# LeCAR-Lab/dial-mpc

Hardware: NVIDIA H100
Metric: sample-steps/s (Nsample*Hsample/wall-s) per MPC reverse_once, Go2 (higher is better)
Workload: dtype f32

## Files before the change

### __graft_entry__.py

```python
from __future__ import annotations

import os
import subprocess
import sys

ROOT = os.path.dirname(os.path.abspath(__file__))
CSRC = os.path.join(ROOT, "dial_mpc_b200", "csrc")
LIB = os.path.join(CSRC, "libdial_b200.so")
NVCC_FLAGS = ["-gencode", "arch=compute_90a,code=sm_90a", "-lineinfo", "-O3", "-std=c++17",
              "-use_fast_math", "-Xcompiler", "-fPIC"]
LINK_FLAGS = ["-gencode", "arch=compute_90a,code=sm_90a", "-shared", "-Xcompiler", "-fPIC", "-cudart", "static"]
VARIANTS = (1, 2, 3, 4, 0)
OBJDIR = os.path.join(CSRC, "build")


def _digest(srcs, extra=""):
    import hashlib
    h = hashlib.sha256()
    for s in srcs:
        h.update(open(s, "rb").read())
    h.update((" ".join(NVCC_FLAGS + LINK_FLAGS) + extra).encode())
    return h.hexdigest()


def _stale(target, digest):
    side = target + ".sha256"
    if not (os.path.exists(target) and os.path.exists(side)):
        return True
    return open(side).read().strip() != digest


def _stamp(target, digest):
    with open(target + ".sha256", "w") as f:
        f.write(digest)


def _shape_defines():
    if ROOT not in sys.path:
        sys.path.insert(0, ROOT)
    from dial_mpc_b200.modelc.shape import SHAPES, env_structure_defines
    return [(name, env_structure_defines(env)) for name, env in SHAPES]


def build_library(force: bool = False, extra=(), lib: str = LIB, objdir: str = OBJDIR) -> None:
    extra = list(extra)
    tag = " " + " ".join(extra)
    hdrs = [os.path.join(CSRC, f) for f in ("dial_device.cuh", "dial_host.h")] + [os.path.join(ROOT, "include", "dial_b200.h")]
    var_src = os.path.join(CSRC, "dial_rollout_variant.cu")
    abi_src = os.path.join(CSRC, "dial_kernels.cu")
    shapes = _shape_defines()
    shape_tag = "".join(f" {name}:" + ",".join(d) for name, d in shapes)
    lib_digest = _digest(hdrs + [var_src, abi_src], tag + shape_tag)
    if not (force or _stale(lib, lib_digest)):
        return
    nvcc = os.environ.get("NVCC", "/usr/local/cuda/bin/nvcc")
    os.makedirs(objdir, exist_ok=True)
    jobs = []
    for v in VARIANTS:
        obj = os.path.join(objdir, f"rollout_v{v}.o")
        jobs.append((obj, _digest(hdrs + [var_src], f" variant={v}" + tag),
                     [nvcc] + NVCC_FLAGS + extra + [f"-DDIAL_VARIANT={v}", "-c", "-o", obj, var_src]))
    for name, defs in shapes:
        obj = os.path.join(objdir, f"rollout_{name}.o")
        flags = ["-DDIAL_VARIANT=1", f"-DDIAL_SHAPE_NAME={name}"] + [f"-D{d}" for d in defs]
        jobs.append((obj, _digest(hdrs + [var_src], " " + " ".join(flags) + tag),
                     [nvcc] + NVCC_FLAGS + extra + flags + ["-c", "-o", obj, var_src]))
    obj = os.path.join(objdir, "dial_kernels.o")
    jobs.append((obj, _digest(hdrs + [abi_src], tag), [nvcc] + NVCC_FLAGS + extra + ["-c", "-o", obj, abi_src]))
    running = [(o, d, subprocess.Popen(cmd)) for o, d, cmd in jobs if force or _stale(o, d)]
    for o, d, p in running:
        if p.wait() != 0:
            for _, _, q in running:
                q.wait()
            raise RuntimeError(f"nvcc failed for {o}")
        _stamp(o, d)
    subprocess.check_call([nvcc] + LINK_FLAGS + ["-o", lib] + [o for o, _, _ in jobs])
    _stamp(lib, lib_digest)


def build(force: bool = False) -> None:
    build_library(force)
    if ROOT not in sys.path:
        sys.path.insert(0, ROOT)
    import dial_mpc_b200
    from dial_mpc_b200 import _capi
    _capi.lib()
    ex = os.path.join(ROOT, "dial_mpc_b200", "examples", "custom_env")
    if ex not in sys.path:
        sys.path.insert(0, ex)
    import quadpod_env
    _ = quadpod_env.QuadpodEnv(quadpod_env.QuadpodEnvConfig()).library_path
    from dial_mpc_b200 import custom
    custom.build_library(quadpod_env.QuadpodEnv.reward_source, variant=0)
    import pincher_env
    _ = pincher_env.PincherEnv(pincher_env.PincherEnvConfig()).library_path
    for mod in ("tests.emul.emul", "oracle.build_oracle"):
        path = os.path.join(ROOT, *mod.split(".")) + ".py"
        if os.path.exists(path):
            subprocess.check_call([sys.executable, "-c", f"import {mod} as m; m.build()"], cwd=ROOT)


def smoke() -> None:
    if ROOT not in sys.path:
        sys.path.insert(0, ROOT)
    import numpy as np
    import torch
    build()
    import dial_mpc_b200.envs as E
    from dial_mpc_b200 import random as drandom
    from dial_mpc_b200.core.dial_config import DialConfig
    from dial_mpc_b200.core.dial_core import MBDPI
    from oracle.envs_oracle import make_env
    from oracle.planner_oracle import PlannerOracle
    torch.cuda.set_device(0)
    cfg = DialConfig(env_name="unitree_go2_walk", Nsample=64, Hsample=8, Hnode=4, temp_sample=0.05)
    env = E.get_environment(cfg.env_name, config=E.UnitreeGo2EnvConfig(default_vx=0.8, ramp_up_time=1.0))
    mb = MBDPI(cfg, env)
    state = env.reset(drandom.PRNGKey(0))
    rng = np.random.default_rng(0)
    eps = rng.standard_normal((cfg.Nsample, cfg.Hnode + 1, mb.nu)).astype(np.float32)
    Y0 = torch.zeros(cfg.Hnode + 1, mb.nu, device=mb.device)
    _, Ybar, info = mb.reverse_once(state, drandom.PRNGKey(1), Y0, mb.sigma_control, eps=eps)
    torch.cuda.synchronize()
    o = make_env(cfg.env_name, dict(default_vx=0.8, ramp_up_time=1.0))
    po = PlannerOracle(o, cfg.Nsample, cfg.Hsample, cfg.Hnode, cfg.temp_sample, cfg.horizon_diffuse_factor,
                       cfg.traj_diffuse_factor)
    Yo, io = po.reverse_once(o.reset(), eps.astype(np.float64), np.zeros((cfg.Hnode + 1, mb.nu)), po.sigma_control)
    rews = info["rews"].cpu().numpy()
    err_r = np.abs(rews - io["rews"]).max()
    err_y = np.abs(Ybar.cpu().numpy() - Yo).max()
    print(f"smoke: max|rews - oracle| = {err_r:.3e}, max|Ybar - oracle| = {err_y:.3e}, launches = {mb.plan.launches}")
    assert np.isfinite(rews).all()
    assert err_r < 2e-3 and err_y < 5e-3, "CUDA reverse_once disagrees with the oracle"


if __name__ == "__main__":
    build()
    if len(sys.argv) > 1 and sys.argv[1] == "smoke":
        smoke()
```

### dial_mpc_b200/csrc/dial_kernels.cu

```cuda
#include <cuda_runtime.h>
#include <stdio.h>
#include <stdlib.h>
#include <float.h>
#include <cmath>
#include <memory>
#include <string>
#include <vector>
#include <new>
#include "dial_host.h"
#define DIAL_STR2(x) #x
#define DIAL_STR(x) DIAL_STR2(x)

static thread_local std::string g_err;
static int fail(const std::string& s) { g_err = s; return -1; }
#define CUDA_OK(x) do { cudaError_t e_ = (x); if (e_ != cudaSuccess) return fail(std::string(#x) + ": " + cudaGetErrorString(e_)); } while (0)

#ifdef DIAL_ONLY_VARIANT
#define DIAL_HAS_VARIANT(v) ((v) == DIAL_ONLY_VARIANT)
#define DIAL_VARIANT DIAL_ONLY_VARIANT
#include "dial_rollout_variant.cu"
#else
#define DIAL_HAS_VARIANT(v) 1
#endif
#define DIAL_DECL_LAUNCH(v) cudaError_t dial_launch_rollout_v##v(const DevModel*, const DevPlan*, const RolloutArgs&, int, int, size_t, cudaStream_t);
#if DIAL_HAS_VARIANT(0)
DIAL_DECL_LAUNCH(0)
#endif
#if DIAL_HAS_VARIANT(1)
DIAL_DECL_LAUNCH(1)
#endif
#if DIAL_HAS_VARIANT(2)
DIAL_DECL_LAUNCH(2)
#endif
#if DIAL_HAS_VARIANT(3)
DIAL_DECL_LAUNCH(3)
#endif
#if DIAL_HAS_VARIANT(4)
DIAL_DECL_LAUNCH(4)
#endif
#ifndef DIAL_ONLY_VARIANT
typedef cudaError_t (*dial_launch_fn)(const DevModel*, const DevPlan*, const RolloutArgs&, int, int, size_t, cudaStream_t);
#define DIAL_DECL_SHAPE(s) \
  cudaError_t dial_launch_rollout_##s(const DevModel*, const DevPlan*, const RolloutArgs&, int, int, size_t, cudaStream_t); \
  bool dial_shape_matches_##s(const DevModel&, const dial_plan_desc&);
DIAL_DECL_SHAPE(go2)
static const struct {
  const char* name;
  dial_launch_fn launch;
  bool (*matches)(const DevModel&, const dial_plan_desc&);
} kShapes[] = {{"go2", dial_launch_rollout_go2, dial_shape_matches_go2}};
#endif

template <typename T, int K>
__device__ __forceinline__ void block_reduce(T (&v)[K], T* mx, T* red) {
  const int lane = threadIdx.x & 31, wid = threadIdx.x >> 5, nw = blockDim.x >> 5;
#pragma unroll
  for (int o = 16; o > 0; o >>= 1) {
#pragma unroll
    for (int k = 0; k < K; ++k) v[k] += __shfl_xor_sync(0xffffffffu, v[k], o);
    if (mx) *mx = fmax(*mx, __shfl_xor_sync(0xffffffffu, *mx, o));
  }
  __syncthreads();
  if (lane == 0) {
#pragma unroll
    for (int k = 0; k < K; ++k) red[k * 32 + wid] = v[k];
    if (mx) red[K * 32 + wid] = *mx;
  }
  __syncthreads();
#pragma unroll
  for (int k = 0; k < K; ++k) v[k] = lane < nw ? red[k * 32 + lane] : T(0);
  if (mx) *mx = lane < nw ? red[K * 32 + lane] : T(-INFINITY);
#pragma unroll
  for (int o = 16; o > 0; o >>= 1) {
#pragma unroll
    for (int k = 0; k < K; ++k) v[k] += __shfl_xor_sync(0xffffffffu, v[k], o);
    if (mx) *mx = fmax(*mx, __shfl_xor_sync(0xffffffffu, *mx, o));
  }
}

struct SoftmaxParams {
  float shift, inv, mx;
  bool none;
};
__device__ __noinline__ SoftmaxParams reward_softmax_params_fp64(const float* __restrict__ rews, int n, float temp,
                                                                 float rbar, float mean, float cnt, float* red_f) {
  double* red = reinterpret_cast<double*>(red_f);
  SoftmaxParams s;
  s.none = false;
  const double c = isfinite(mean) ? (double)rbar + (double)mean : 0.0;
  double s1[1] = {0.0}, s2[1] = {0.0}, rmax = -INFINITY;
  for (int i = threadIdx.x; i < n; i += blockDim.x) {
    const float r = __ldcg(rews + i);
    if (isfinite(r)) { const double d = (double)r - c; s1[0] += d; s2[0] += d * d; rmax = fmax(rmax, (double)r); }
  }
  block_reduce<double, 1>(s1, &rmax, red);
  block_reduce<double, 1>(s2, nullptr, red);
  const double m = s1[0] / (double)cnt, var64 = s2[0] / (double)cnt - m * m;
  s.shift = (float)rmax;
  s.mx = 0.f;
  s.inv = var64 > 0.0 ? (float)fmin(1.0 / (sqrt(var64) * (double)temp), 3.4028234663852886e38) : 0.f;
  return s;
}
__device__ __forceinline__ SoftmaxParams reward_softmax_params(const float* __restrict__ rews, int n, float temp,
                                                               float* red) {
  float rbar = __ldcg(rews + n - 1);
  const bool rbar_finite = isfinite(rbar);
  if (!rbar_finite) rbar = 0.f;
  float st[3] = {0.f, 0.f, 0.f}, dmax = -INFINITY;
  for (int i = threadIdx.x; i < n; i += blockDim.x) {
    const float r = __ldcg(rews + i);
    if (isfinite(r)) { const float d = r - rbar; st[0] += 1.f; st[1] += d; st[2] += d * d; dmax = fmaxf(dmax, d); }
  }
  block_reduce<float, 3>(st, &dmax, red);
  SoftmaxParams s;
  const float cnt = st[0];
  s.none = cnt == 0.f;
  const float mean = st[1] / fmaxf(cnt, 1.f);
  const float var = st[2] / fmaxf(cnt, 1.f) - mean * mean;
  const float sd = sqrtf(fmaxf(var, 0.f));
  if (s.none || (rbar_finite && isfinite(st[2]) && fabsf(mean) <= 8.f * sd)) {
    s.shift = rbar;
    s.inv = (sd > 0.f) ? 1.f / sd / temp : 0.f;
    s.mx = dmax * s.inv;
    return s;
  }
  return reward_softmax_params_fp64(rews, n, temp, rbar, mean, cnt, red);
}

struct XchWait {
  const float* mbox;
  const uint32_t* flags;
  uint32_t* seq;
  uint32_t* err;
  float* rews_copy;
  int world;
};
__device__ __forceinline__ unsigned long long globaltimer_ns() {
  unsigned long long t;
  asm volatile("mov.u64 %0, %%globaltimer;" : "=l"(t));
  return t;
}
__device__ __forceinline__ void xch_wait_flags(const uint32_t* flags, uint32_t want, int world, uint32_t* err,
                                               uint32_t* acc = nullptr) {
  if ((int)threadIdx.x < world) {
    const volatile uint32_t* f = flags + threadIdx.x;
    const unsigned long long t0 = globaltimer_ns();
    while (*f < want) {
      if (globaltimer_ns() - t0 > 4000000000ull) { *err = 1u; break; }
      __nanosleep(100);
    }
    if (acc) {
      const unsigned long long dt = globaltimer_ns() - t0;
      const unsigned m = __reduce_max_sync(__activemask(), (unsigned)(dt > 0xffffffffull ? 0xffffffffull : dt));
      if (threadIdx.x == 0) *acc += m;
    }
    __threadfence_system();
  }
  __syncthreads();
}

__global__ void __launch_bounds__(1024) weights_kernel(const float* __restrict__ rews, int n, float temp,
                                                        float* __restrict__ weights, const XchWait X) {
  __shared__ __align__(8) float red[4 * 32];
  const int tid = threadIdx.x;
  if (X.mbox) {
    const uint32_t seq = *X.seq, buf = seq & 1u;
    xch_wait_flags(X.flags + buf * DIAL_MAXRANK, seq + 1u, X.world, X.err, X.err + 2);
    rews = X.mbox + (size_t)buf * n;
    if (X.rews_copy)
      for (int i = tid; i < n; i += blockDim.x) X.rews_copy[i] = __ldcg(rews + i);
  }
  const SoftmaxParams s = reward_softmax_params(rews, n, temp, red);
  if (s.none) {
    for (int i = tid; i < n; i += blockDim.x) weights[i] = (i == n - 1) ? 1.f : 0.f;
    if (X.mbox && tid == 0) *X.seq = *X.seq + 1u;
    return;
  }
  float z[1] = {0.f};
  for (int i = tid; i < n; i += blockDim.x) {
    const float r = __ldcg(rews + i);
    const float e = isfinite(r) ? expf((r - s.shift) * s.inv - s.mx) : 0.f;
    weights[i] = e;
    z[0] += e;
  }
  block_reduce<float, 1>(z, nullptr, red);
  const float iz = 1.f / z[0];
  for (int i = tid; i < n; i += blockDim.x) weights[i] *= iz;
  if (X.mbox && tid == 0) *X.seq = *X.seq + 1u;
}

struct BarsXch {
  float* mbox[DIAL_MAXRANK];
  uint32_t* flags[DIAL_MAXRANK];
  uint32_t* seq;
  uint32_t* err;
  int world, rank, nbar;
  const float* partial;
  float* out[3];
  int n0, n1;
};
__global__ void __launch_bounds__(1024) bars_allreduce_kernel(const BarsXch B) {
  const uint32_t seq = *B.seq, buf = seq & 1u;
  const size_t half = (size_t)buf * DIAL_MAXRANK * B.nbar;
  for (int p = 0; p < B.world; ++p) {
    float* dst = B.mbox[p] + half + (size_t)B.rank * B.nbar;
    for (int i = threadIdx.x; i < B.nbar; i += blockDim.x) dst[i] = B.partial[i];
  }
  __threadfence_system();
  __syncthreads();
  if (threadIdx.x == 0) {
    __threadfence_system();
    for (int p = 0; p < B.world; ++p)
      *reinterpret_cast<volatile uint32_t*>(B.flags[p] + buf * DIAL_MAXRANK + B.rank) = seq + 1u;
  }
  __syncthreads();
  xch_wait_flags(B.flags[B.rank] + buf * DIAL_MAXRANK, seq + 1u, B.world, B.err, B.err + 3);
  const float* mine = B.mbox[B.rank] + half;
  for (int i = threadIdx.x; i < B.nbar; i += blockDim.x) {
    float s_ = 0.f;
    for (int p = 0; p < B.world; ++p) s_ += __ldcg(mine + (size_t)p * B.nbar + i);
    float* o = i < B.n0 ? B.out[0] + i : (i < B.n0 + B.n1 ? B.out[1] + (i - B.n0) : B.out[2] + (i - B.n0 - B.n1));
    *o = s_;
  }
  __syncthreads();
  if (threadIdx.x == 0) *B.seq = seq + 1u;
}

__device__ __forceinline__ float ordered_column_sum(const float* __restrict__ col, int stride, unsigned count, bool on) {
  float tot = 0.f;
  if (!on) return tot;
  unsigned b = 0;
  for (; b + 16 <= count; b += 16) {
    float v[16];
#pragma unroll
    for (int k = 0; k < 16; ++k) v[k] = __ldcg(col + (size_t)(b + k) * stride);
#pragma unroll
    for (int k = 0; k < 16; ++k) tot += v[k];
  }
  for (; b < count; ++b) tot += __ldcg(col + (size_t)b * stride);
  return tot;
}

#define YBAR_THREADS 256
__global__ void __launch_bounds__(YBAR_THREADS) ybar_kernel(const float* __restrict__ weights, const float* __restrict__ eps,
                                                             uint32_t key0, uint32_t key1, const float* __restrict__ Ybar,
                                                             const float* __restrict__ noise, int Ntotal, int Hn1, int nu,
                                                             float* __restrict__ partial, unsigned int* __restrict__ counter,
                                                             float* __restrict__ Ybar_out,
                                                             const uint32_t* __restrict__ key_dev) {
  if (key_dev) { key0 = key_dev[0]; key1 = key_dev[1]; }
  const int ne = Hn1 * nu;
  __shared__ float acc[YBAR_THREADS];
  __shared__ bool is_last;
  const int slots = YBAR_THREADS / ne;
  const int slot = threadIdx.x / ne, el = threadIdx.x - slot * ne;
  float a = 0.f;
  if (slot < slots) {
    const int k = el / nu;
    const float yb = Ybar[el], ns = noise[k];
    const uint32_t ntot = (uint32_t)Ntotal * (uint32_t)ne;
    for (int n = blockIdx.x * slots + slot; n <= Ntotal; n += gridDim.x * slots) {
      float y = yb;
      if (n < Ntotal && k > 0) {
        uint32_t idx = (uint32_t)n * (uint32_t)ne + (uint32_t)el;
        float e = eps ? eps[idx] : jax_normal_legacy(key0, key1, idx, ntot);
        y = e * ns + yb;
      }
      y = fminf(fmaxf(y, -1.f), 1.f);
      a += weights[n] * y;
    }
  }
  acc[threadIdx.x] = a;
  __syncthreads();
  if (threadIdx.x < ne) {
    float s = 0.f;
    for (int sl = 0; sl < slots; ++sl) s += acc[sl * ne + threadIdx.x];
    partial[blockIdx.x * ne + threadIdx.x] = s;
  }
  __threadfence();
  __syncthreads();
  if (threadIdx.x == 0) is_last = (atomicAdd(counter, 1u) == gridDim.x - 1);
  __syncthreads();
  if (is_last) {
    if (threadIdx.x < ne) Ybar_out[threadIdx.x] = ordered_column_sum(partial + threadIdx.x, ne, gridDim.x, true);
    if (threadIdx.x == 0) *counter = 0u;
  }
}

__global__ void __launch_bounds__(YBAR_THREADS) update_kernel(const float* __restrict__ rews, int n, float temp,
                                                               float* __restrict__ weights, const XchWait X,
                                                               uint32_t* __restrict__ rng, const float* __restrict__ Ybar,
                                                               const float* __restrict__ noise, int Ntotal, int Hn1, int nu,
                                                               float* __restrict__ partial, unsigned int* __restrict__ counter,
                                                               float* __restrict__ Ybar_out, const InstSchedule* __restrict__ sched,
                                                               const int32_t* __restrict__ iter_lim, int iter,
                                                               const float* weights_prev) {
  __shared__ __align__(8) float red[4 * 32];
  __shared__ float acc[YBAR_THREADS];
  __shared__ bool is_last;
  const int tid = threadIdx.x;
  {
    const size_t b = blockIdx.y, ne1 = (size_t)Hn1 * nu;
    rews += b * n; weights += b * n; rng += 2 * b; Ybar += b * ne1; Ybar_out += b * ne1;
    partial += b * gridDim.x * (ne1 + 1); counter += b;
    if (!schedule_runs(iter_lim, b, iter)) {
      if (blockIdx.x == 0)
        for (int i = tid; i < (int)ne1; i += blockDim.x) Ybar_out[i] = Ybar[i];
      if (weights_prev != weights - b * n)
        for (int i = blockIdx.x * blockDim.x + tid; i < n; i += gridDim.x * blockDim.x) weights[i] = weights_prev[b * n + i];
      return;
    }
    if (sched && sched[b].on) { temp = sched[b].temp; noise = sched[b].noise[iter]; }
  }
  if (X.mbox) {
    const uint32_t seq = *X.seq, buf = seq & 1u;
    xch_wait_flags(X.flags + buf * DIAL_MAXRANK, seq + 1u, X.world, X.err, blockIdx.x == 0 ? X.err + 2 : nullptr);
    rews = X.mbox + (size_t)buf * n;
  }
  uint32_t key0, key1;
  const uint32_t r0 = rng[0], r1 = rng[1];
  split_key(r0, r1, key0, key1);
  const SoftmaxParams sp = reward_softmax_params(rews, n, temp, red);
  const int ne = Hn1 * nu;
  const int slots = YBAR_THREADS / ne;
  const int slot = tid / ne, el = tid - slot * ne;
  float a = 0.f, z = 0.f;
  if (slot < slots) {
    const int k = el / nu;
    const float yb = Ybar[el], ns = noise[k];
    const uint32_t ntot = (uint32_t)Ntotal * (uint32_t)ne;
    for (int s_ = blockIdx.x * slots + slot; s_ <= Ntotal; s_ += gridDim.x * slots) {
      const float r = __ldcg(rews + s_);
      float e = isfinite(r) ? expf((r - sp.shift) * sp.inv - sp.mx) : 0.f;
      if (sp.none) e = (s_ == Ntotal) ? 1.f : 0.f;
      float y = yb;
      if (s_ < Ntotal && k > 0) {
        const uint32_t idx = (uint32_t)s_ * (uint32_t)ne + (uint32_t)el;
        y = jax_normal_legacy(key0, key1, idx, ntot) * ns + yb;
      }
      y = fminf(fmaxf(y, -1.f), 1.f);
      a += e * y;
      if (el == 0) { z += e; weights[s_] = e; }
    }
  }
  acc[tid] = a;
  float zz[1] = {z};
  block_reduce<float, 1>(zz, nullptr, red);
  __syncthreads();
  if (tid < ne) {
    float s_ = 0.f;
    for (int sl = 0; sl < slots; ++sl) s_ += acc[sl * ne + tid];
    partial[blockIdx.x * (ne + 1) + tid] = s_;
  }
  if (tid == 0) partial[blockIdx.x * (ne + 1) + ne] = zz[0];
  __threadfence();
  __syncthreads();
  if (tid == 0) is_last = (atomicAdd(counter, 1u) == gridDim.x - 1);
  __syncthreads();
  if (!is_last) return;
  __threadfence();
  __shared__ float zsh;
  float tot = ordered_column_sum(partial + tid, ne + 1, gridDim.x, tid <= ne);
  if (tid == ne) zsh = tot;
  if (ne == (int)blockDim.x && tid == 0) zsh = ordered_column_sum(partial + ne, ne + 1, gridDim.x, true);
  __syncthreads();
  const float iz = 1.f / zsh;
  if (tid < ne) Ybar_out[tid] = tot * iz;
  for (int i = tid; i < n; i += blockDim.x) {
    weights[i] = __ldcg(weights + i) * iz;
    if (X.mbox && X.rews_copy) X.rews_copy[i] = __ldcg(rews + i);
  }
  if (tid == 0) {
    *counter = 0u;
    uint32_t n0, n1;
    split_rng(r0, r1, n0, n1);
    rng[0] = n0; rng[1] = n1;
    if (X.mbox) *X.seq = *X.seq + 1u;
  }
}

__global__ void mpc_split_kernel(uint32_t* __restrict__ rng, uint32_t* __restrict__ key) {
  if (threadIdx.x == 0) {
    const uint32_t k0 = rng[0], k1 = rng[1];
    uint32_t a0 = 0, b0 = 2, a1 = 1, b1 = 3;
    threefry2x32(k0, k1, a0, b0);
    threefry2x32(k0, k1, a1, b1);
    rng[0] = a0; rng[1] = a1; key[0] = b0; key[1] = b1;
  }
}

__global__ void mpc_shift_kernel(const float* __restrict__ Msh, const float* __restrict__ Yin,
                                 float* __restrict__ Yout, int n1, int nu) {
  const int i = threadIdx.x;
  Yin += (size_t)blockIdx.x * n1 * nu; Yout += (size_t)blockIdx.x * n1 * nu;
  if (i < n1 * nu) {
    const int k = i / nu, a = i - k * nu;
    float s = 0.f;
    for (int j = 0; j < n1; ++j) s += Msh[k * n1 + j] * Yin[j * nu + a];
    Yout[i] = s;
  }
}

#define TB_CHUNKS 32
struct TrajArgs {
  const float* traj[3];
  float* out[3];
  int ncol[3], coloff[3];
  int coltot, nrows, H;
  int inst_rows;
  const float* weights;
  int w_offset, mean_row, mean_weight_index, include_mean;
  float* partial;
};

template <bool BATCH>
__global__ void __launch_bounds__(256, 8) trajbar_partial_kernel(const TrajArgs T, const int32_t* __restrict__ iter_lim, int iter) {
  const int chunk = blockIdx.y, arr = BATCH ? blockIdx.z % 3 : blockIdx.z, inst = BATCH ? blockIdx.z / 3 : 0;
  const int ncol = arr == 0 ? T.ncol[0] : (arr == 1 ? T.ncol[1] : T.ncol[2]), len = T.H * ncol;
  const int coloff = arr == 0 ? T.coloff[0] : (arr == 1 ? T.coloff[1] : T.coloff[2]);
  const int j = blockIdx.x * 256 + threadIdx.x;
  if (blockIdx.x * 256 >= len || (BATCH && !schedule_runs(iter_lim, inst, iter))) return;
  const float* __restrict__ traj = (arr == 0 ? T.traj[0] : (arr == 1 ? T.traj[1] : T.traj[2])) + (size_t)inst * T.inst_rows * len;
  const float* wts = BATCH ? T.weights + (size_t)inst * (T.mean_weight_index + 1) : T.weights;
  const int per = (T.nrows + TB_CHUNKS - 1) / TB_CHUNKS;
  const int r0 = chunk * per, r1 = min(T.nrows, r0 + per);
  const int jj = j < len ? j : len - 1;
  float a = 0.f;
  for (int r = r0; r < r1; r += 8) {
    float wv[8], xv[8];
#pragma unroll
    for (int k = 0; k < 8; ++k) {
      const int rr = r + k;
      float wgt = 0.f;
      if (rr < r1) {
        if (rr == T.mean_row) wgt = T.include_mean ? wts[T.mean_weight_index] : 0.f;
        else wgt = wts[T.w_offset + rr];
      }
      wv[k] = wgt;
    }
#pragma unroll
    for (int k = 0; k < 8; ++k)
      xv[k] = (wv[k] != 0.f) ? traj[(size_t)(r + k) * len + jj] : 0.f;
#pragma unroll
    for (int k = 0; k < 8; ++k) a += wv[k] * xv[k];
  }
  if (j < len) {
    const int t = j / ncol, c = j - t * ncol;
    T.partial[(((size_t)inst * TB_CHUNKS + chunk) * T.H + t) * T.coltot + coloff + c] = a;
  }
}

template <bool BATCH>
__global__ void __launch_bounds__(128, 8) trajbar_final_kernel(const TrajArgs T, const int32_t* __restrict__ iter_lim, int iter) {
  const int t = blockIdx.x, inst = BATCH ? blockIdx.y : 0;
  if (BATCH && !schedule_runs(iter_lim, inst, iter)) return;
  const float* partial = T.partial + (size_t)inst * TB_CHUNKS * T.H * T.coltot;
  for (int col = threadIdx.x; col < T.coltot; col += blockDim.x) {
    float s = 0.f;
#pragma unroll 8
    for (int ch = 0; ch < TB_CHUNKS; ++ch) s += partial[((size_t)ch * T.H + t) * T.coltot + col];
    float* out; int ncol, off;
    if (col >= T.coloff[2]) { out = T.out[2]; ncol = T.ncol[2]; off = T.coloff[2]; }
    else if (col >= T.coloff[1]) { out = T.out[1]; ncol = T.ncol[1]; off = T.coloff[1]; }
    else { out = T.out[0]; ncol = T.ncol[0]; off = T.coloff[0]; }
    if (out) out[((size_t)inst * T.H + t) * ncol + (col - off)] = s;
  }
}

__global__ void __launch_bounds__(256) ensemble_reduce_kernel(const float* __restrict__ r, const EnsRisk* __restrict__ risk,
                                                              const EnsAdapt* __restrict__ adapt, const float* __restrict__ belief,
                                                              int K, int n1, float* __restrict__ rews,
                                                              const int32_t* __restrict__ iter_lim, int iter) {
  const int i = blockIdx.x * blockDim.x + threadIdx.x, b = blockIdx.y;
  if (i >= n1 || !schedule_runs(iter_lim, b, iter)) return;
  const EnsRisk R = risk[b];
  const float* rb = r + (size_t)b * K * n1 + i;
  rews[(size_t)b * n1 + i] = adapt[b].on ? ens_risk_reduce_weighted(rb, (size_t)n1, K, R, belief + (size_t)b * K, adapt[b].prune)
                                         : ens_risk_reduce(rb, (size_t)n1, K, R);
}

__global__ void __launch_bounds__(128) ens_gather_kernel(const float* __restrict__ Y, int K, int n1, int nu,
                                                         float* __restrict__ us) {
  const int b = blockIdx.x;
  for (int i = threadIdx.x; i < K * nu; i += blockDim.x) us[(size_t)b * K * nu + i] = Y[(size_t)b * n1 * nu + i % nu];
}

__global__ void __launch_bounds__(32) ens_belief_kernel(const float* __restrict__ vhat, const float* __restrict__ qvel,
                                                        const EnsAdapt* __restrict__ adapt, int K, int nv,
                                                        double* __restrict__ L, float* __restrict__ w, float* __restrict__ ell) {
  const int b = blockIdx.x, lane = threadIdx.x;
  if (!adapt[b].on) return;
  __shared__ double l[DIAL_MAXENS];
  if (lane < K) {
    l[lane] = ens_member_loglik(vhat + ((size_t)b * K + lane) * nv, qvel + (size_t)b * nv, adapt[b].sigma, nv);
    ell[(size_t)b * K + lane] = (float)l[lane];
  }
  __syncwarp();
  if (lane == 0) ens_belief_update(L + (size_t)b * K, w + (size_t)b * K, l, K, (double)adapt[b].forget);
}

__global__ void __launch_bounds__(128) delay_queue_kernel(const DelaySetting* __restrict__ set, int32_t* __restrict__ head,
                                                          float* __restrict__ ring, const float* __restrict__ Y, int n1,
                                                          int nu, int pop, float* __restrict__ applied,
                                                          float* __restrict__ pending, int32_t* __restrict__ pred_len) {
  const int b = blockIdx.x;
  const DelaySetting s = set[b];
  const int h = head[b];
  const size_t q = (size_t)b * DIAL_MAXDELAY * nu;
  const int h1 = delay_queue_step(ring + q, h, s.d, nu, Y + (size_t)b * n1 * nu, applied + (size_t)b * nu, pending + q,
                                  pop != 0, threadIdx.x, blockDim.x);
  __syncthreads();
  if (threadIdx.x == 0) { head[b] = h1; pred_len[b] = s.predict && s.d > 0 ? s.d : 0; }
}

__global__ void __launch_bounds__(128) delay_refill_kernel(int b, int d, int32_t* __restrict__ head, float* __restrict__ ring,
                                                           const float* __restrict__ Y, int n1, int nu,
                                                           float* __restrict__ pending) {
  const size_t q = (size_t)b * DIAL_MAXDELAY * nu;
  const float* y0 = Y + (size_t)b * n1 * nu;
  for (int a = threadIdx.x; a < nu; a += blockDim.x)
    for (int j = 0; j < d; ++j) ring[q + (size_t)j * nu + a] = y0[a];
  delay_queue_step(ring + q, 0, d, nu, y0, nullptr, pending + q, false, threadIdx.x, blockDim.x);
  if (threadIdx.x == 0) head[b] = 0;
}

struct ObsBuffers {
  ObsRing* ring;
  float *rq, *rv, *rw, *ra;
  int32_t* rc;
  float *oq, *ov, *ow;
  int32_t *oc, *age;
  float* seq;
  int32_t* len;
};

__global__ void __launch_bounds__(128) observe_kernel(const DevModel* __restrict__ M, const ObsSetting* __restrict__ set,
                                                      ObsBuffers O, const DelaySetting* __restrict__ dset,
                                                      const float* __restrict__ pending, int env_step,
                                                      const float* __restrict__ qpos, const float* __restrict__ qvel,
                                                      const float* __restrict__ warm, const int32_t* __restrict__ cnt,
                                                      const float* __restrict__ act, int act_row, float* __restrict__ pq,
                                                      float* __restrict__ pv, float* __restrict__ pw, int32_t* __restrict__ pc) {
  const int b = blockIdx.x;
  const dial_model_desc& m = M->m;
  const size_t nq = m.nq, nv = m.nv, nu = m.nu, R = DIAL_OBSRING;
  const ObsSetting& s = set[b];
  const ObsRing r = O.ring[b];
  const DelaySetting ds = dset ? dset[b] : DelaySetting{0, 0};
  const ObsRing r1 = observe_advance(s, r, env_step != 0);
  ObsView V;
  V.qpos = qpos + b * nq; V.qvel = qvel + b * nv; V.warm = warm + b * nv; V.cnt = cnt + 2 * b;
  V.act = env_step ? act + b * act_row : nullptr;
  V.rq = O.rq + b * R * nq; V.rv = O.rv + b * R * nv; V.rw = O.rw + b * R * nv; V.ra = O.ra + b * R * nu;
  V.rc = O.rc + b * R * 2;
  V.oq = O.oq + b * nq; V.ov = O.ov + b * nv; V.ow = O.ow + b * nv; V.oc = O.oc + 2 * b;
  V.pq = pq + b * nq; V.pv = pv + b * nv; V.pw = pw + b * nv; V.pc = pc + 2 * b;
  V.seq = O.seq + b * DIAL_MAXDELAY * nu;
  V.pending = pending ? pending + b * DIAL_MAXDELAY * nu : nullptr;
  observe_record(observe_pushes(s, r, env_step != 0), r1, V, (int)nq, (int)nv, (int)nu, threadIdx.x, blockDim.x);
  __syncthreads();
  observe_emit(s, r1, m, ds.d, V, threadIdx.x, blockDim.x);
  if (threadIdx.x == 0) {
    const int age = observe_age(s, r1);
    O.ring[b] = r1; O.age[b] = age; O.len[b] = ds.predict ? age + ds.d : 0;
  }
}

__global__ void observe_reset_kernel(int b, const ObsSetting* __restrict__ set, ObsRing* __restrict__ ring) {
  ObsRing r;
  r.head = 0; r.count = 0;
  r.key[0] = set[b].key[0]; r.key[1] = set[b].key[1]; r.sub[0] = 0u; r.sub[1] = 0u;
  ring[b] = r;
}

template <class T> struct Staged {
  T* d = nullptr;
  T* h = nullptr;
  size_t width = 1;
  std::vector<cudaEvent_t> ev;
  cudaError_t allocate(size_t n, size_t w, const T& init) {
    width = w;
    cudaError_t e = cudaMallocHost(&h, n * w * sizeof(T));
    if (e == cudaSuccess) e = cudaMalloc(&d, n * w * sizeof(T));
    if (e == cudaSuccess) {
      for (size_t i = 0; i < n * w; ++i) h[i] = init;
      e = cudaMemcpy(d, h, n * w * sizeof(T), cudaMemcpyHostToDevice);
    }
    if (e != cudaSuccess) { release(); return e; }
    ev.assign(n, nullptr);
    return cudaSuccess;
  }
  template <class F> cudaError_t put(size_t s, F fill, cudaStream_t st) {
    cudaEvent_t& e_s = ev[s];
    cudaError_t e = e_s ? cudaEventSynchronize(e_s) : cudaEventCreateWithFlags(&e_s, cudaEventDisableTiming);
    if (e == cudaSuccess) {
      fill(h + s * width);
      e = cudaMemcpyAsync(d + s * width, h + s * width, width * sizeof(T), cudaMemcpyHostToDevice, st);
    }
    if (e == cudaSuccess) e = cudaEventRecord(e_s, st);
    return e;
  }
  void release() {
    for (cudaEvent_t e : ev) if (e) cudaEventDestroy(e);
    ev.clear();
    cudaFree(d); cudaFreeHost(h);
    d = nullptr; h = nullptr;
  }
};

struct LaunchKey {
  bool models = false, members = false, sched = false, lims = false, adapt = false, delay = false, obs = false;
  bool predicts = false;
  int npred = 0;
  bool planning() const { return obs || npred > 0; }
  bool operator!=(const LaunchKey& o) const {
    return models != o.models || members != o.members || sched != o.sched || lims != o.lims || adapt != o.adapt ||
           delay != o.delay || obs != o.obs || predicts != o.predicts || npred != o.npred;
  }
};

struct dial_plan {
  DevModel hM;
  DevPlan hP;
  DevModel* dM = nullptr;
  DevPlan* dP = nullptr;
  int variant = 0;
  int shape = 0;
  int n_inst = 1;
  int n_ens = 0;
  int num_sms = 132;
  size_t smem_bytes = 0;
  float *traj_q[2] = {nullptr, nullptr}, *traj_qd[2] = {nullptr, nullptr}, *traj_x[2] = {nullptr, nullptr};
  int cur = 0;
  float* weights = nullptr;
  float* weights2 = nullptr;
  cudaStream_t side = nullptr;
  cudaEvent_t ev_main[2] = {nullptr, nullptr}, ev_side[2] = {nullptr, nullptr};
  float* partial = nullptr;
  float* tb_partial = nullptr;
  unsigned int* counter = nullptr;
  unsigned int* row_counter = nullptr;
  float* zeros = nullptr;
  int ybar_grid = 0;
  int upd_grid = 0;
  int64_t launches = 0;
  float* dbg = nullptr;
  dial_mpc_buffers mpc{};
  bool mpc_bound = false;
  float* mpc_Msh = nullptr;
  float* mpc_Y1 = nullptr;
  uint32_t* mpc_key = nullptr;
  struct MpcGraph { int n_diffuse, env_step, seen; cudaGraphExec_t exec; int64_t launches; };
  std::vector<MpcGraph> mpc_graphs;
  LaunchKey key, ran;
  Staged<DevModel> models;
  Staged<DevModel> members;
  float* ens_rews = nullptr;
  Staged<EnsRisk> risk;
  Staged<EnsAdapt> adapt;
  Staged<double> belief_L;
  Staged<float> belief_w;
  float* dEll = nullptr;
  float* pred_us = nullptr;
  float* pred_qd = nullptr;
  Staged<InstSchedule> sched;
  Staged<int32_t> lims;
  struct PlanningState {
    float *qpos = nullptr, *qvel = nullptr, *warm = nullptr;
    int32_t* cnt = nullptr;
    DevModel* models = nullptr;
  } planning;
  Staged<DelaySetting> delay;
  struct DelayQueue {
    int32_t* head = nullptr;
    float *ring = nullptr, *applied = nullptr, *pending = nullptr;
    int32_t* len = nullptr;
  } queue;
  Staged<ObsSetting> obs;
  ObsBuffers ob{};
  std::vector<void**> owned;
  template <class T> cudaError_t own(cudaError_t& e, T*& ptr, size_t bytes, bool zero = false, cudaStream_t st = nullptr) {
    void** slot = reinterpret_cast<void**>(&ptr);
    if (e == cudaSuccess && (e = cudaMalloc(slot, bytes)) == cudaSuccess) owned.push_back(slot);
    if (e == cudaSuccess && zero) e = cudaMemsetAsync(ptr, 0, bytes, st);
    return e;
  }
  void free_since(size_t mark) {
    for (; owned.size() > mark; owned.pop_back()) { cudaFree(*owned.back()); *owned.back() = nullptr; }
  }
  struct Exchange {
    bool on = false;
    int rank = 0, world = 1, nbar = 0;
    uint32_t* base[DIAL_MAXRANK] = {nullptr};
    size_t words = 0, o_mbox = 0, o_bars = 0, o_flags = 0, o_bflags = 0, o_local = 0;
    float* bars_partial = nullptr;
    float* mbox(int p) const { return reinterpret_cast<float*>(base[p] + o_mbox); }
    float* bars(int p) const { return reinterpret_cast<float*>(base[p] + o_bars); }
    uint32_t* flags(int p) const { return base[p] + o_flags; }
    uint32_t* bflags(int p) const { return base[p] + o_bflags; }
    uint32_t* seq() const { return base[rank] + o_local; }
    unsigned int* done() const { return base[rank] + o_local + 1; }
    uint32_t* err() const { return base[rank] + o_local + 2; }
    uint32_t* bseq() const { return base[rank] + o_local + 3; }
  } xch;
};

static void drop_graphs(dial_plan* p) {
  for (auto& g : p->mpc_graphs) if (g.exec) cudaGraphExecDestroy(g.exec);
  p->mpc_graphs.clear();
}

static LaunchKey launch_key(const dial_plan* p) {
  LaunchKey k;
  k.models = p->models.d != nullptr; k.members = p->members.d != nullptr;
  k.sched = p->sched.d != nullptr; k.lims = p->lims.d != nullptr; k.adapt = p->pred_qd != nullptr;
  k.delay = p->delay.d != nullptr; k.obs = p->obs.d != nullptr;
  for (int b = 0; k.delay && b < p->n_inst; ++b) {
    const DelaySetting& s = p->delay.h[b];
    const int n = s.d + (k.obs && p->obs.h[b].on ? p->obs.h[b].k : 0);
    if (!s.predict) continue;
    k.predicts |= s.d > 0;
    k.npred = n > k.npred ? n : k.npred;
  }
  return k;
}

static void fill_xch(const dial_plan* p, RolloutArgs& A) {
  if (!p->xch.on) return;
  A.xch_world = p->xch.world; A.xch_rank = p->xch.rank;
  for (int r = 0; r < p->xch.world; ++r) { A.xch_mbox[r] = p->xch.mbox(r); A.xch_flags[r] = p->xch.flags(r); }
  A.xch_seq = p->xch.seq(); A.xch_done = p->xch.done();
}
static XchWait xch_wait_args(const dial_plan* p, float* rews_copy) {
  XchWait X; memset(&X, 0, sizeof(X));
  if (p->xch.on) {
    X.mbox = p->xch.mbox(p->xch.rank); X.flags = p->xch.flags(p->xch.rank); X.seq = p->xch.seq(); X.err = p->xch.err();
    X.rews_copy = rews_copy; X.world = p->xch.world;
  }
  return X;
}

extern "C" int dial_abi_version(void) { return DIAL_ABI_VERSION; }
extern "C" const char* dial_last_error(void) { return g_err.c_str(); }
extern "C" size_t dial_sizeof(int which) {
  return which == 0 ? sizeof(dial_model_desc) : which == 1 ? sizeof(dial_plan_desc) : which == 2 ? sizeof(dial_state)
       : which == 3 ? sizeof(dial_mpc_buffers) : which == 4 ? sizeof(dial_task) : 0;
}

static cudaError_t launch_rollout(dial_plan* p, const RolloutArgs& A, int wpc, cudaStream_t st) {
  const size_t smem = sizeof(DevModel) + sizeof(DevPlan) + (size_t)wpc * p->hM.warp_floats * sizeof(float);
  int grid = (A.nrows + wpc - 1) / wpc;
  if (A.models && model_rows(A) > 0) grid = (A.nrows / model_rows(A)) * ((model_rows(A) + wpc - 1) / wpc);
  if (A.row_counter) {
    const int resident = p->num_sms * (wpc > 8 ? 1 : 16 / wpc);
    grid = grid < resident ? grid : resident;
    cudaError_t e = cudaMemsetAsync(A.row_counter, 0, sizeof(unsigned int), st);
    if (e != cudaSuccess) return e;
  }
  p->launches++;
#ifndef DIAL_ONLY_VARIANT
  if (p->shape > 0) return kShapes[p->shape - 1].launch(p->dM, p->dP, A, grid, wpc, smem, st);
#endif
  switch (p->variant) {
#if DIAL_HAS_VARIANT(1)
    case 1: return dial_launch_rollout_v1(p->dM, p->dP, A, grid, wpc, smem, st);
#endif
#if DIAL_HAS_VARIANT(2)
    case 2: return dial_launch_rollout_v2(p->dM, p->dP, A, grid, wpc, smem, st);
#endif
#if DIAL_HAS_VARIANT(3)
    case 3: return dial_launch_rollout_v3(p->dM, p->dP, A, grid, wpc, smem, st);
#endif
#if DIAL_HAS_VARIANT(4)
    case 4: return dial_launch_rollout_v4(p->dM, p->dP, A, grid, wpc, smem, st);
#endif
#if DIAL_HAS_VARIANT(0)
    case 0: return dial_launch_rollout_v0(p->dM, p->dP, A, grid, wpc, smem, st);
#endif
    default: return cudaErrorInvalidDeviceFunction;
  }
}

static int default_wpc(const dial_plan* p, int nrows) {
  const int per_sm = (nrows + p->num_sms - 1) / p->num_sms;
  const size_t fixed = sizeof(DevModel) + sizeof(DevPlan), slab = (size_t)p->hM.warp_floats * sizeof(float);
  int maxw = DIAL_MAXTHREADS / 32;
  while (maxw > 1 && fixed + maxw * slab > 227 * 1024) --maxw;
  if (per_sm <= maxw) return per_sm;
  const int waves = (per_sm + maxw - 1) / maxw;
  return (per_sm + waves - 1) / waves;
}

static cudaError_t launch_rollout_any(dial_plan* p, const RolloutArgs& A0, cudaStream_t st) {
  RolloutArgs A = A0;
  const char* f = getenv("DIAL_WPC");
  int wpc = f ? atoi(f) : 0;
  if (wpc == 0) {
    wpc = default_wpc(p, A.nrows);
    if (A.models && model_rows(A) > 0) {
      const int cpi = (model_rows(A) + wpc - 1) / wpc;
      wpc = (model_rows(A) + cpi - 1) / cpi;
    }
  }
  if (wpc < 1 || wpc > DIAL_MAXTHREADS / 32) return cudaErrorInvalidValue;
  A.lockstep = (wpc >= 2 && !getenv("DIAL_NO_LOCKSTEP")) ? 1 : 0;
  if (p->hM.dense && !A.lockstep && !A.models && A.nrows > wpc * p->num_sms && !getenv("DIAL_NO_DYNAMIC_ROWS")) A.row_counter = p->row_counter;
  const bool mid = getenv("DIAL_MIDSYNC") ? true : (getenv("DIAL_NO_MIDSYNC") ? false : (p->hM.dense || !p->hM.s_on));
  if (A.lockstep && mid) A.lockstep = 2;
  { const char* se = getenv("DIAL_SYNC_EVERY"); A.sync_every = se ? atoi(se) : 1; if (A.sync_every < 1) A.sync_every = 1; }
  const char* dl = getenv("DIAL_DENSE_LOCKSTEP");
  if (A.lockstep == 2 && p->hM.dense && !(dl && atoi(dl) == 2)) A.lockstep = 3;
  return launch_rollout(p, A, wpc, st);
}

extern "C" dial_plan* dial_plan_create(const dial_model_desc* model, const dial_plan_desc* cfg) {
  if (!model || !cfg) { g_err = "null descriptor"; return nullptr; }
  dial_plan* p = new (std::nothrow) dial_plan();
  if (!p) { g_err = "out of memory"; return nullptr; }
  std::string err;
  if (!derive_model(*model, p->hM, err)) { g_err = err; delete p; return nullptr; }
  {
    int dev = 0, sms = 0;
    if (cudaGetDevice(&dev) == cudaSuccess && cudaDeviceGetAttribute(&sms, cudaDevAttrMultiProcessorCount, dev) == cudaSuccess && sms > 0)
      p->num_sms = sms;
  }
  p->variant = (getenv("DIAL_FORCE_GENERIC_TREE") && !p->hM.dense) ? 0 : star_variant(p->hM);
  if (p->variant < 0) { g_err = "this build instantiates the dense (elliptic) solver path for nv = " DIAL_STR(DIAL_DENSE_NV) " only (custom builds: dial_mpc_b200.custom compiles it for the model's nv)"; delete p; return nullptr; }
  memset(&p->hP, 0, sizeof(DevPlan));
  p->hP.c = *cfg;
  p->hP.c.cmd_step = -1;
  const dial_plan_desc& c = *cfg;
  if (c.Hsample + 1 > DIAL_MAXH || c.Hnode + 1 > DIAL_MAXNODE || c.Hnode < 1 || c.Nsample < 1 || c.Ntotal < c.Nsample ||
      c.n_frames < 1 || (c.Hnode + 1) * model->nu > YBAR_THREADS || c.n_stage > DIAL_MAXSTAGE) {
    g_err = "invalid plan configuration (Hsample/Hnode/Nsample/n_frames out of range)";
    delete p;
    return nullptr;
  }
  if (c.env_id < DIAL_ENV_GO2_WALK || c.env_id > DIAL_ENV_CUSTOM) { g_err = "unknown env_id"; delete p; return nullptr; }
#ifndef DIAL_CUSTOM_REWARD_FILE
  if (c.env_id == DIAL_ENV_CUSTOM) {
    g_err = "env_id DIAL_ENV_CUSTOM needs a library built with a reward source (dial_mpc_b200.custom.build_library); this is the stock build";
    delete p; return nullptr;
  }
#endif
#ifdef DIAL_ONLY_VARIANT
  if (p->variant != DIAL_ONLY_VARIANT) {
    g_err = "this custom build holds solver variant " + std::to_string(DIAL_ONLY_VARIANT) + " only, the model needs " + std::to_string(p->variant);
    delete p; return nullptr;
  }
#endif
  if (c.n_user < 0 || c.n_user > DIAL_MAXUSER) { g_err = "n_user out of range"; delete p; return nullptr; }
  if (c.n_inst < 0) { g_err = "n_inst must be >= 0 (0 or 1: a single instance)"; delete p; return nullptr; }
  if (c.n_inst > 1) {
    if (c.Ntotal != c.Nsample) { g_err = "a batched plan (n_inst > 1) cannot be sharded (Ntotal must equal Nsample)"; delete p; return nullptr; }
    if (c.Nsample + 1 > (1 << 17)) { g_err = "a batched plan (n_inst > 1) needs Nsample + 1 <= 131072 (the fused update)"; delete p; return nullptr; }
    if (c.n_inst > 65535 / 3 || (int64_t)c.n_inst * (c.Nsample + 1) > 0x7fffffff) {
      g_err = "n_inst too large: at most 21845 instances and 2^31 - 1 rows per rollout launch"; delete p; return nullptr;
    }
  }
  p->n_inst = c.n_inst > 1 ? c.n_inst : 1;
  if (c.n_ens < 0 || c.n_ens > DIAL_MAXENS) { g_err = "n_ens out of range (0..DIAL_MAXENS = " DIAL_STR(DIAL_MAXENS) ")"; delete p; return nullptr; }
  if (c.n_ens >= 1) {
    if (c.Ntotal != c.Nsample) { g_err = "an ensemble plan (n_ens >= 1) cannot be sharded (Ntotal must equal Nsample)"; delete p; return nullptr; }
    if ((int64_t)p->n_inst * c.n_ens * (c.Nsample + 1) > 0x7fffffff) { g_err = "n_inst * n_ens * (Nsample + 1) exceeds 2^31 - 1 rows per rollout launch"; delete p; return nullptr; }
  }
  p->n_ens = c.n_ens;
#ifndef DIAL_ONLY_VARIANT
  if (p->variant == 1 && !getenv("DIAL_FORCE_GENERIC_SHAPE"))
    for (int s = 0; s < (int)(sizeof(kShapes) / sizeof(kShapes[0])); ++s)
      if (kShapes[s].matches(p->hM, p->hP.c)) { p->shape = s + 1; break; }
#endif
  auto bad = [&](cudaError_t e, const char* what) {
    g_err = std::string(what) + ": " + cudaGetErrorString(e);
    dial_plan_destroy(p);
    return (dial_plan*)nullptr;
  };
  cudaError_t e = cudaSuccess;
  if (p->own(e, p->dM, sizeof(DevModel)) != cudaSuccess) return bad(e, "cudaMalloc(model)");
  if (p->own(e, p->dP, sizeof(DevPlan)) != cudaSuccess) return bad(e, "cudaMalloc(plan)");
  if ((e = cudaMemcpy(p->dM, &p->hM, sizeof(DevModel), cudaMemcpyHostToDevice)) != cudaSuccess) return bad(e, "cudaMemcpy(model)");
  if ((e = cudaMemcpy(p->dP, &p->hP, sizeof(DevPlan), cudaMemcpyHostToDevice)) != cudaSuccess) return bad(e, "cudaMemcpy(plan)");
  const size_t B = (size_t)p->n_inst, H = (size_t)c.Hsample + 1;
  const size_t rows = B * (p->n_ens > 1 ? (size_t)p->n_ens : 1) * ((size_t)c.Nsample + 1);
  const dial_model_desc& m = *model;
  for (int b = 0; b < 2; ++b) {
    if (p->own(e, p->traj_q[b], rows * H * m.nq * sizeof(float)) != cudaSuccess) return bad(e, "cudaMalloc(traj_q)");
    if (p->own(e, p->traj_qd[b], rows * H * m.nv * sizeof(float)) != cudaSuccess) return bad(e, "cudaMalloc(traj_qd)");
    if (p->own(e, p->traj_x[b], rows * H * 3 * (m.nbody - 1) * sizeof(float)) != cudaSuccess) return bad(e, "cudaMalloc(traj_x)");
  }
  if (p->n_ens > 1) {
    if (p->own(e, p->ens_rews, rows * sizeof(float)) != cudaSuccess) return bad(e, "cudaMalloc(ens_rews)");
    const size_t K = p->n_ens;
    const double L0 = log(1.0 / p->n_ens);
    if ((e = p->risk.allocate(B, 1, ens_risk_derive(p->n_ens, DIAL_ENS_MEAN, 1.f))) != cudaSuccess) return bad(e, "allocate(risk)");
    if ((e = p->adapt.allocate(B, 1, EnsAdapt{})) != cudaSuccess) return bad(e, "allocate(adapt)");
    if ((e = p->belief_L.allocate(B, K, L0)) != cudaSuccess) return bad(e, "allocate(belief)");
    if ((e = p->belief_w.allocate(B, K, (float)exp(L0))) != cudaSuccess) return bad(e, "allocate(belief)");
    if (p->own(e, p->dEll, B * K * sizeof(float)) != cudaSuccess) return bad(e, "cudaMalloc(belief)");
    if ((e = cudaMemset(p->dEll, 0, B * K * sizeof(float))) != cudaSuccess) return bad(e, "cudaMemset(belief)");
  }
  if (p->own(e, p->weights, B * ((size_t)c.Ntotal + 1) * sizeof(float)) != cudaSuccess) return bad(e, "cudaMalloc(weights)");
  if (p->own(e, p->weights2, B * ((size_t)c.Ntotal + 1) * sizeof(float)) != cudaSuccess) return bad(e, "cudaMalloc(weights2)");
  if ((e = cudaStreamCreateWithFlags(&p->side, cudaStreamNonBlocking)) != cudaSuccess) return bad(e, "cudaStreamCreate(side)");
  for (int i = 0; i < 2; ++i) {
    if ((e = cudaEventCreateWithFlags(&p->ev_main[i], cudaEventDisableTiming)) != cudaSuccess) return bad(e, "cudaEventCreate");
    if ((e = cudaEventCreateWithFlags(&p->ev_side[i], cudaEventDisableTiming)) != cudaSuccess) return bad(e, "cudaEventCreate");
  }
  const int ne = (c.Hnode + 1) * m.nu, slots = YBAR_THREADS / ne;
  int g = (c.Ntotal + 1 + slots - 1) / slots;
  p->ybar_grid = g < 1 ? 1 : (g > 2 * p->num_sms ? 2 * p->num_sms : g);
  {
    int gu = (c.Ntotal + 1 + slots * 8 - 1) / (slots * 8);
    p->upd_grid = gu < 1 ? 1 : (gu > p->ybar_grid ? p->ybar_grid : gu);
  }
  if (p->own(e, p->partial, B * p->ybar_grid * (ne + 1) * sizeof(float)) != cudaSuccess) return bad(e, "cudaMalloc(partial)");
  if (p->own(e, p->tb_partial, B * TB_CHUNKS * H * (m.nq + m.nv + 3 * (m.nbody - 1)) * sizeof(float)) != cudaSuccess) return bad(e, "cudaMalloc(tb_partial)");
  if (p->own(e, p->counter, B * sizeof(unsigned int)) != cudaSuccess) return bad(e, "cudaMalloc(counter)");
  if ((e = cudaMemset(p->counter, 0, B * sizeof(unsigned int))) != cudaSuccess) return bad(e, "cudaMemset(counter)");
  if (p->own(e, p->row_counter, sizeof(unsigned int)) != cudaSuccess) return bad(e, "cudaMalloc(row_counter)");
  if (getenv("DIAL_DEBUG_COUNTERS")) {
    if (p->own(e, p->dbg, 8 * sizeof(float)) != cudaSuccess) return bad(e, "cudaMalloc(dbg)");
    cudaMemset(p->dbg, 0, 8 * sizeof(float));
  }
  if (p->own(e, p->zeros, DIAL_MAXV * sizeof(float)) != cudaSuccess) return bad(e, "cudaMalloc(zeros)");
  if ((e = cudaMemset(p->zeros, 0, DIAL_MAXV * sizeof(float))) != cudaSuccess) return bad(e, "cudaMemset(zeros)");
  return p;
}

extern "C" void dial_plan_destroy(dial_plan* p) {
  if (!p) return;
  drop_graphs(p);
  for (int r = 0; r < DIAL_MAXRANK; ++r) {
    if (!p->xch.base[r]) continue;
    if (r == p->xch.rank) cudaFree(p->xch.base[r]); else cudaIpcCloseMemHandle(p->xch.base[r]);
  }
  cudaFree(p->xch.bars_partial);
  p->models.release(); p->members.release(); p->risk.release();
  p->adapt.release(); p->belief_L.release(); p->belief_w.release(); p->sched.release(); p->lims.release();
  p->delay.release(); p->obs.release();
  for (int i = 0; i < 2; ++i) { if (p->ev_main[i]) cudaEventDestroy(p->ev_main[i]); if (p->ev_side[i]) cudaEventDestroy(p->ev_side[i]); }
  if (p->side) cudaStreamDestroy(p->side);
  p->free_since(0);
  delete p;
}

static void fill_state(RolloutArgs& A, const dial_state* s) {
  A.qpos0 = s->qpos; A.qvel0 = s->qvel; A.warm0 = s->qacc_warmstart; A.step0 = s->step; A.stage0 = s->stage;
}

extern "C" int dial_rollout(dial_plan* p, const dial_state* s, const float* us, int B, int H, float* rewss,
                            float* q, float* qd, float* xpos, void* stream) {
  if (!p || !s || !us || !rewss) return fail("dial_rollout: null argument");
  if (B < 1 || H < 1) return fail("dial_rollout: B and H must be positive");
  RolloutArgs A; memset(&A, 0, sizeof(A));
  fill_state(A, s);
  A.nrows = B; A.H = H; A.mode = 0; A.us = us; A.rewss = rewss; A.q = q; A.qd = qd; A.xpos = xpos;
  CUDA_OK(launch_rollout_any(p, A, (cudaStream_t)stream));
  return 0;
}

extern "C" int dial_plan_set_command(dial_plan* p, int cmd_step, const float* vel, const float* ang, void* stream) {
  if (!p) return fail("dial_plan_set_command: null plan");
  if (cmd_step >= 0 && (!vel || !ang)) return fail("dial_plan_set_command: null command");
  dial_plan_desc& c = p->hP.c;
  c.cmd_step = cmd_step;
  for (int i = 0; i < 3; ++i) { c.cmd_vel[i] = cmd_step >= 0 ? vel[i] : 0.f; c.cmd_ang[i] = cmd_step >= 0 ? ang[i] : 0.f; }
  const size_t off = offsetof(dial_plan_desc, cmd_step);
  CUDA_OK(cudaMemcpyAsync((char*)p->dP + off, (const char*)&p->hP.c + off, sizeof(int32_t) + 6 * sizeof(float),
                          cudaMemcpyHostToDevice, (cudaStream_t)stream));
  return 0;
}

extern "C" int dial_plan_set_stages(dial_plan* p, int n_stage, const float* pose_seq, const float* yaw_seq,
                                    const float* contact_targets, const float* contact_radius, void* stream) {
  if (!p) return fail("dial_plan_set_stages: null plan");
  if (n_stage < 1 || n_stage > DIAL_MAXSTAGE) return fail("dial_plan_set_stages: n_stage out of range (1..DIAL_MAXSTAGE)");
  if (!pose_seq || !yaw_seq || !contact_targets || !contact_radius) return fail("dial_plan_set_stages: null table");
  dial_plan_desc& c = p->hP.c;
  c.n_stage = n_stage;
  memset(c.pose_seq, 0, sizeof(c.pose_seq)); memset(c.yaw_seq, 0, sizeof(c.yaw_seq));
  memset(c.contact_targets, 0, sizeof(c.contact_targets)); memset(c.contact_radius, 0, sizeof(c.contact_radius));
  memcpy(c.pose_seq, pose_seq, sizeof(float) * 3 * n_stage);
  memcpy(c.yaw_seq, yaw_seq, sizeof(float) * n_stage);
  memcpy(c.contact_targets, contact_targets, sizeof(float) * 12 * n_stage);
  memcpy(c.contact_radius, contact_radius, sizeof(float) * 4 * n_stage);
  const size_t off = offsetof(dial_plan_desc, n_stage), end = offsetof(dial_plan_desc, n_user);
  CUDA_OK(cudaMemcpyAsync((char*)p->dP + off, (const char*)&p->hP.c + off, end - off, cudaMemcpyHostToDevice,
                          (cudaStream_t)stream));
  return 0;
}

static std::string fmt_g(double x) {
  char buf[64];
  snprintf(buf, sizeof(buf), "%g", x);
  return buf;
}

static int need_ensemble(const dial_plan* p, const char* fn, int k) {
  if (!p) return fail(std::string(fn) + ": null plan");
  if (p->n_ens >= k) return 0;
  if (k == 1) return fail(std::string(fn) + ": the plan has no ensemble (dial_plan_desc.n_ens = 0)");
  return fail(std::string(fn) + ": the plan needs an ensemble of n_ens >= " + std::to_string(k) + " members, it has " + std::to_string(p->n_ens));
}
static int need_instance(const dial_plan* p, const char* fn, int b) {
  if (b >= 0 && b < p->n_inst) return 0;
  return fail(std::string(fn) + ": instance " + std::to_string(b) + " out of range (0.." + std::to_string(p->n_inst - 1) + ")");
}

static int set_model_slot(dial_plan* p, const char* fn, Staged<DevModel>& a, size_t n, size_t slot,
                          const dial_model_desc* m, cudaStream_t st) {
  std::unique_ptr<DevModel> D(new (std::nothrow) DevModel());
  if (!D) return fail("out of memory");
  std::string err;
  if (!derive_model(*m, *D, err)) return fail(std::string(fn) + ": " + err);
  if (const char* diff = instance_model_difference(p->hM, *D))
    return fail(std::string(fn) + ": field '" + diff + "' differs from the plan's model "
                "(an instance's model may differ in floats other than timestep, jnt_range and actuator_ctrlrange only)");
  cudaError_t e = cudaSuccess;
  if (!a.d && (e = a.allocate(n, 1, p->hM)) != cudaSuccess) return fail(std::string(fn) + ": " + cudaGetErrorString(e));
  e = a.put(slot, [&](DevModel* h) { *h = *D; }, st);
  p->key = launch_key(p);
  CUDA_OK(e);
  return 0;
}

extern "C" int dial_plan_set_instance_model(dial_plan* p, int b, const dial_model_desc* m, void* stream) {
  static const char* fn = "dial_plan_set_instance_model";
  if (!p || !m) return fail(std::string(fn) + ": null argument");
  if (int rc = need_instance(p, fn, b)) return rc;
  if (p->hP.c.Ntotal != p->hP.c.Nsample) return fail(std::string(fn) + ": sharded plans (Ntotal != Nsample) share one model");
  return set_model_slot(p, fn, p->models, (size_t)p->n_inst, (size_t)b, m, (cudaStream_t)stream);
}

extern "C" int dial_plan_set_ensemble_model(dial_plan* p, int b, int k, const dial_model_desc* m, void* stream) {
  static const char* fn = "dial_plan_set_ensemble_model";
  if (!p || !m) return fail(std::string(fn) + ": null argument");
  if (int rc = need_ensemble(p, fn, 1)) return rc;
  if (int rc = need_instance(p, fn, b)) return rc;
  if (k < 0 || k >= p->n_ens) return fail(std::string(fn) + ": member " + std::to_string(k) + " out of range (0.." + std::to_string(p->n_ens - 1) + ")");
  const size_t slot = (size_t)b * p->n_ens + k;
  if (int rc = set_model_slot(p, fn, p->members, (size_t)p->n_inst * p->n_ens, slot, m, (cudaStream_t)stream)) return rc;
  if (k == 0 && p->planning.models)
    CUDA_OK(cudaMemcpyAsync(p->planning.models + b, p->members.d + slot, sizeof(DevModel), cudaMemcpyDeviceToDevice, (cudaStream_t)stream));
  return 0;
}

extern "C" int dial_plan_set_ensemble_risk(dial_plan* p, int b, int mode, float alpha, void* stream) {
  static const char* fn = "dial_plan_set_ensemble_risk";
  if (int rc = need_ensemble(p, fn, 1)) return rc;
  if (int rc = need_instance(p, fn, b)) return rc;
  if (mode != DIAL_ENS_MEAN && mode != DIAL_ENS_CVAR)
    return fail(std::string(fn) + ": mode " + std::to_string(mode) + " is neither DIAL_ENS_MEAN (0) nor DIAL_ENS_CVAR (1)");
  if (mode == DIAL_ENS_CVAR && !(alpha > 0.f && alpha <= 1.f))
    return fail(std::string(fn) + ": alpha must be finite and in (0, 1] for DIAL_ENS_CVAR, got " + fmt_g(alpha));
  if (p->n_ens < 2) return 0;
  cudaError_t e = p->risk.put(b, [&](EnsRisk* r) { *r = ens_risk_derive(p->n_ens, mode, alpha); }, (cudaStream_t)stream);
  if (e != cudaSuccess) return fail(std::string(fn) + ": " + cudaGetErrorString(e));
  return 0;
}

extern "C" int dial_plan_member_rewards(dial_plan* p, float* out, void* stream) {
  static const char* fn = "dial_plan_member_rewards";
  if (!p || !out) return fail(std::string(fn) + ": null argument");
  if (int rc = need_ensemble(p, fn, 1)) return rc;
  if (!p->mpc_bound) return fail(std::string(fn) + ": call dial_mpc_bind first");
  const size_t n = (size_t)p->n_inst * p->n_ens * ((size_t)p->hP.c.Nsample + 1);
  const float* src = p->n_ens > 1 ? p->ens_rews : p->mpc.rews;
  CUDA_OK(cudaMemcpyAsync(out, src, n * sizeof(float), cudaMemcpyDeviceToDevice, (cudaStream_t)stream));
  return 0;
}

extern "C" int dial_plan_set_ensemble_adapt(dial_plan* p, int b, int on, float forget, float prune, const float* sigma, void* stream) {
  static const char* fn = "dial_plan_set_ensemble_adapt";
  if (int rc = need_ensemble(p, fn, 2)) return rc;
  if (int rc = need_instance(p, fn, b)) return rc;
  if (on != 0 && on != 1) return fail(std::string(fn) + ": on must be 0 or 1, got " + std::to_string(on));
  const int K = p->n_ens, nv = p->hM.m.nv;
  if (on) {
    if (!(forget > 0.f && forget <= 1.f)) return fail(std::string(fn) + ": forget must be in (0, 1], got " + fmt_g(forget));
    if (!(prune >= 0.f && (double)prune < 1.0 / K))
      return fail(std::string(fn) + ": prune must be in [0, 1/K) = [0, " + fmt_g(1.0 / K) + "), got " + fmt_g(prune));
    if (!sigma) return fail(std::string(fn) + ": null sigma");
    for (int j = 0; j < nv; ++j)
      if (!(sigma[j] > 0.f && sigma[j] <= FLT_MAX))
        return fail(std::string(fn) + ": sigma[" + std::to_string(j) + "] must be finite and > 0, got " + fmt_g(sigma[j]));
  }
  cudaStream_t st = (cudaStream_t)stream;
  cudaError_t e = cudaSuccess;
  if (on && !p->pred_qd) {
    const size_t rows = (size_t)p->n_inst * K, mark = p->owned.size();
    p->own(e, p->pred_us, rows * p->hM.m.nu * sizeof(float));
    if (p->own(e, p->pred_qd, rows * nv * sizeof(float)) != cudaSuccess) {
      p->free_since(mark);
      return fail(std::string(fn) + ": " + cudaGetErrorString(e));
    }
  }
  e = p->adapt.put(b, [&](EnsAdapt* a) {
    a->on = on;
    if (on) {
      a->forget = forget; a->prune = prune;
      for (int j = 0; j < DIAL_MAXV; ++j) a->sigma[j] = j < nv ? sigma[j] : 1.f;
    }
  }, st);
  p->key = launch_key(p);
  if (e != cudaSuccess) return fail(std::string(fn) + ": " + cudaGetErrorString(e));
  return 0;
}

extern "C" int dial_plan_set_ensemble_belief(dial_plan* p, int b, const float* w, void* stream) {
  static const char* fn = "dial_plan_set_ensemble_belief";
  if (int rc = need_ensemble(p, fn, 2)) return rc;
  if (int rc = need_instance(p, fn, b)) return rc;
  if (!w) return fail(std::string(fn) + ": null w");
  const int K = p->n_ens;
  double sum = 0.0;
  for (int k = 0; k < K; ++k) {
    if (!(w[k] >= 0.f && w[k] <= FLT_MAX)) return fail(std::string(fn) + ": w[" + std::to_string(k) + "] must be finite and >= 0, got " + fmt_g(w[k]));
    sum += (double)w[k];
  }
  if (!(sum > 0.0)) return fail(std::string(fn) + ": the weights must have a positive sum");
  cudaStream_t st = (cudaStream_t)stream;
  cudaError_t e = p->belief_L.put(b, [&](double* L) {
    for (int k = 0; k < K; ++k) L[k] = w[k] > 0.f ? log((double)w[k] / sum) : -INFINITY;
  }, st);
  const double* L = p->belief_L.h + (size_t)b * K;
  if (e == cudaSuccess) e = p->belief_w.put(b, [&](float* W) {
    for (int k = 0; k < K; ++k) W[k] = (float)exp(L[k]);
  }, st);
  if (e != cudaSuccess) return fail(std::string(fn) + ": " + cudaGetErrorString(e));
  return 0;
}

extern "C" int dial_plan_ensemble_belief(dial_plan* p, float* w, float* loglik, void* stream) {
  if (int rc = need_ensemble(p, "dial_plan_ensemble_belief", 2)) return rc;
  const size_t n = (size_t)p->n_inst * p->n_ens * sizeof(float);
  cudaStream_t st = (cudaStream_t)stream;
  if (w) CUDA_OK(cudaMemcpyAsync(w, p->belief_w.d, n, cudaMemcpyDeviceToDevice, st));
  if (loglik) CUDA_OK(cudaMemcpyAsync(loglik, p->dEll, n, cudaMemcpyDeviceToDevice, st));
  return 0;
}

static int need_schedulable(const dial_plan* p, const char* fn) {
  const dial_plan_desc& c = p->hP.c;
  if (c.Ntotal != c.Nsample) return fail(std::string(fn) + ": sharded plans (Ntotal != Nsample) share the plan's schedule");
  if (c.Ntotal + 1 > (1 << 17)) return fail(std::string(fn) + ": needs Ntotal + 1 <= 131072 (the fused update)");
  return 0;
}

extern "C" int dial_plan_set_instance_schedule(dial_plan* p, int b, float temp, int n_rows, const float* noise, void* stream) {
  static const char* fn = "dial_plan_set_instance_schedule";
  if (!p) return fail(std::string(fn) + ": null plan");
  if (int rc = need_instance(p, fn, b)) return rc;
  if (int rc = need_schedulable(p, fn)) return rc;
  const int n1 = p->hP.c.Hnode + 1;
  if (noise) {
    if (!(temp > 0.f && temp <= FLT_MAX)) return fail(std::string(fn) + ": temp must be finite and > 0, got " + fmt_g(temp));
    if (n_rows < 1 || n_rows > DIAL_MAXDIFFUSE)
      return fail(std::string(fn) + ": n_rows " + std::to_string(n_rows) + " out of range (1.." DIAL_STR(DIAL_MAXDIFFUSE) ")");
    for (int i = 0; i < n_rows * n1; ++i)
      if (!(fabsf(noise[i]) <= FLT_MAX))
        return fail(std::string(fn) + ": noise[" + std::to_string(i / n1) + "][" + std::to_string(i % n1) + "] is not finite, got " + fmt_g(noise[i]));
  } else if (!p->sched.d) {
    return 0;
  }
  cudaStream_t st = (cudaStream_t)stream;
  cudaError_t e = cudaSuccess;
  if (!p->sched.d && (e = p->sched.allocate(p->n_inst, 1, InstSchedule{})) != cudaSuccess)
    return fail(std::string(fn) + ": " + cudaGetErrorString(e));
  e = p->sched.put(b, [&](InstSchedule* S) {
    memset(S, 0, sizeof(*S));
    if (!noise) return;
    S->on = 1; S->temp = temp; S->n_rows = n_rows;
    for (int r = 0; r < n_rows; ++r)
      for (int k = 0; k < n1; ++k) S->noise[r][k] = noise[r * n1 + k];
  }, st);
  p->key = launch_key(p);
  if (e != cudaSuccess) return fail(std::string(fn) + ": " + cudaGetErrorString(e));
  return 0;
}

extern "C" int dial_plan_set_instance_iterations(dial_plan* p, const int32_t* n_iter, void* stream) {
  static const char* fn = "dial_plan_set_instance_iterations";
  if (!p || !n_iter) return fail(std::string(fn) + ": null argument");
  if (int rc = need_schedulable(p, fn)) return rc;
  for (int b = 0; b < p->n_inst; ++b)
    if (n_iter[b] < 0 || n_iter[b] > DIAL_MAXDIFFUSE)
      return fail(std::string(fn) + ": n_iter[" + std::to_string(b) + "] = " + std::to_string(n_iter[b]) + " out of range (0.." DIAL_STR(DIAL_MAXDIFFUSE) ")");
  cudaStream_t st = (cudaStream_t)stream;
  cudaError_t e = cudaSuccess;
  if (!p->lims.d) {
    Staged<DevModel>& M = p->n_ens > 0 ? p->members : p->models;
    if (!M.d) e = M.allocate((size_t)p->n_inst * (p->n_ens > 0 ? p->n_ens : 1), 1, p->hM);
    if (e == cudaSuccess) e = p->lims.allocate(1, p->n_inst, DIAL_MAXDIFFUSE);
    if (e != cudaSuccess) return fail(std::string(fn) + ": " + cudaGetErrorString(e));
  }
  e = p->lims.put(0, [&](int32_t* L) { memcpy(L, n_iter, sizeof(int32_t) * p->n_inst); }, st);
  p->key = launch_key(p);
  if (e != cudaSuccess) return fail(std::string(fn) + ": " + cudaGetErrorString(e));
  return 0;
}

static cudaError_t allocate_planning(dial_plan* p, cudaStream_t st) {
  dial_plan::PlanningState& P = p->planning;
  if (P.qpos) return cudaSuccess;
  const size_t B = (size_t)p->n_inst, nq = p->hM.m.nq, nv = p->hM.m.nv;
  cudaError_t e = cudaSuccess;
  p->own(e, P.qpos, B * nq * sizeof(float), true, st);
  p->own(e, P.qvel, B * nv * sizeof(float), true, st);
  p->own(e, P.warm, B * nv * sizeof(float), true, st);
  p->own(e, P.cnt, B * 2 * sizeof(int32_t), true, st);
  if (p->n_ens > 0) p->own(e, P.models, B * sizeof(DevModel));
  for (size_t b = 0; P.models && b < B && e == cudaSuccess; ++b)
    e = p->members.d ? cudaMemcpyAsync(P.models + b, p->members.d + b * p->n_ens, sizeof(DevModel), cudaMemcpyDeviceToDevice, st)
                     : cudaMemcpy(P.models + b, &p->hM, sizeof(DevModel), cudaMemcpyHostToDevice);
  return e;
}

static cudaError_t allocate_delay(dial_plan* p, cudaStream_t st) {
  const size_t B = (size_t)p->n_inst, nu = p->hM.m.nu, mark = p->owned.size();
  dial_plan::DelayQueue& Q = p->queue;
  cudaError_t e = allocate_planning(p, st);
  if (e == cudaSuccess) e = p->delay.allocate(B, 1, DelaySetting{0, 0});
  p->own(e, Q.head, B * sizeof(int32_t), true, st);
  p->own(e, Q.ring, B * DIAL_MAXDELAY * nu * sizeof(float), true, st);
  p->own(e, Q.applied, B * nu * sizeof(float), true, st);
  p->own(e, Q.pending, B * DIAL_MAXDELAY * nu * sizeof(float), true, st);
  p->own(e, Q.len, B * sizeof(int32_t), true, st);
  if (e != cudaSuccess) { p->delay.release(); p->free_since(mark); }
  return e;
}

static cudaError_t allocate_observation(dial_plan* p, cudaStream_t st) {
  const size_t B = (size_t)p->n_inst, nq = p->hM.m.nq, nv = p->hM.m.nv, nu = p->hM.m.nu, R = DIAL_OBSRING;
  const size_t mark = p->owned.size();
  cudaError_t e = allocate_planning(p, st);
  ObsSetting off;
  memset(&off, 0, sizeof(off));
  if (e == cudaSuccess) e = p->obs.allocate(B, 1, off);
  ObsBuffers& O = p->ob;
  p->own(e, O.ring, B * sizeof(ObsRing), true, st);
  p->own(e, O.rq, B * R * nq * sizeof(float), true, st);
  p->own(e, O.rv, B * R * nv * sizeof(float), true, st);
  p->own(e, O.rw, B * R * nv * sizeof(float), true, st);
  p->own(e, O.ra, B * R * nu * sizeof(float), true, st);
  p->own(e, O.rc, B * R * 2 * sizeof(int32_t), true, st);
  p->own(e, O.oq, B * nq * sizeof(float), true, st);
  p->own(e, O.ov, B * nv * sizeof(float), true, st);
  p->own(e, O.ow, B * nv * sizeof(float), true, st);
  p->own(e, O.oc, B * 2 * sizeof(int32_t), true, st);
  p->own(e, O.age, B * sizeof(int32_t), true, st);
  p->own(e, O.seq, B * DIAL_MAXDELAY * nu * sizeof(float), true, st);
  p->own(e, O.len, B * sizeof(int32_t), true, st);
  if (e != cudaSuccess) { p->obs.release(); p->free_since(mark); }
  return e;
}

extern "C" int dial_plan_set_instance_delay(dial_plan* p, int b, int steps, int predict, void* stream) {
  static const char* fn = "dial_plan_set_instance_delay";
  if (!p) return fail(std::string(fn) + ": null plan");
  if (int rc = need_instance(p, fn, b)) return rc;
  const dial_plan_desc& c = p->hP.c;
  if (c.Ntotal != c.Nsample || p->xch.on) return fail(std::string(fn) + ": sharded plans (Ntotal != Nsample) have no per-instance delay");
  if (steps < 0 || steps > DIAL_MAXDELAY)
    return fail(std::string(fn) + ": steps " + std::to_string(steps) + " out of range (0.." DIAL_STR(DIAL_MAXDELAY) ")");
  if (predict != 0 && predict != 1) return fail(std::string(fn) + ": predict must be 0 or 1, got " + std::to_string(predict));
  if (p->obs.d && steps + p->obs.h[b].k > DIAL_MAXDELAY)
    return fail(std::string(fn) + ": steps " + std::to_string(steps) + " plus instance " + std::to_string(b) +
                "'s observation delay " + std::to_string(p->obs.h[b].k) + " exceeds " DIAL_STR(DIAL_MAXDELAY));
  if (!p->mpc_bound) return fail(std::string(fn) + ": call dial_mpc_bind first (the queue is filled from the bound Y)");
  cudaStream_t st = (cudaStream_t)stream;
  cudaError_t e = cudaSuccess;
  if (!p->delay.d && (e = allocate_delay(p, st)) != cudaSuccess) return fail(std::string(fn) + ": " + cudaGetErrorString(e));
  e = p->delay.put(b, [&](DelaySetting* s) { s->d = steps; s->predict = predict; }, st);
  p->key = launch_key(p);
  if (e != cudaSuccess) return fail(std::string(fn) + ": " + cudaGetErrorString(e));
  const int n1 = c.Hnode + 1, nu = p->hM.m.nu;
  delay_refill_kernel<<<1, 128, 0, st>>>(b, steps, p->queue.head, p->queue.ring, p->mpc.Y, n1, nu, p->queue.pending);
  CUDA_OK(cudaGetLastError());
  return 0;
}

extern "C" int dial_plan_set_instance_observation(dial_plan* p, int b, int delay, const float* qpos_std,
                                                  const float* qvel_std, const uint32_t key[2], void* stream) {
  static const char* fn = "dial_plan_set_instance_observation";
  if (!p) return fail(std::string(fn) + ": null plan");
  if (int rc = need_instance(p, fn, b)) return rc;
  if (delay < 0 || delay > DIAL_MAXDELAY)
    return fail(std::string(fn) + ": delay " + std::to_string(delay) + " out of range (0.." DIAL_STR(DIAL_MAXDELAY) ")");
  const int d = p->delay.d ? p->delay.h[b].d : 0;
  if (delay + d > DIAL_MAXDELAY)
    return fail(std::string(fn) + ": delay " + std::to_string(delay) + " plus instance " + std::to_string(b) +
                "'s action delay " + std::to_string(d) + " exceeds " DIAL_STR(DIAL_MAXDELAY));
  const int nv = p->hM.m.nv;
  bool noisy = false;
  for (int w = 0; w < 2; ++w) {
    const float* sd = w == 0 ? qpos_std : qvel_std;
    for (int i = 0; sd && i < nv; ++i) {
      if (!(sd[i] >= 0.f) || !std::isfinite(sd[i]))
        return fail(std::string(fn) + ": " + (w == 0 ? "qpos_std[" : "qvel_std[") + std::to_string(i) + "] = " +
                    std::to_string(sd[i]) + " must be finite and >= 0");
      noisy |= sd[i] != 0.f;
    }
  }
  const dial_plan_desc& c = p->hP.c;
  if (c.Ntotal != c.Nsample || p->xch.on) return fail(std::string(fn) + ": sharded plans (Ntotal != Nsample) have no per-instance observation");
  if (!p->mpc_bound) return fail(std::string(fn) + ": call dial_mpc_bind first");
  cudaStream_t st = (cudaStream_t)stream;
  cudaError_t e = cudaSuccess;
  if (!p->obs.d && (e = allocate_observation(p, st)) != cudaSuccess) return fail(std::string(fn) + ": " + cudaGetErrorString(e));
  e = p->obs.put(b, [&](ObsSetting* s) {
    s->k = delay; s->on = delay > 0 || noisy;
    s->key[0] = key ? key[0] : 0u; s->key[1] = key ? key[1] : 0u;
    for (int i = 0; i < 2 * DIAL_MAXV; ++i) s->sigma[i] = 0.f;
    for (int i = 0; i < nv; ++i) { s->sigma[i] = qpos_std ? qpos_std[i] : 0.f; s->sigma[nv + i] = qvel_std ? qvel_std[i] : 0.f; }
  }, st);
  p->key = launch_key(p);
  if (e != cudaSuccess) return fail(std::string(fn) + ": " + cudaGetErrorString(e));
  observe_reset_kernel<<<1, 1, 0, st>>>(b, p->obs.d, p->ob.ring);
  CUDA_OK(cudaGetLastError());
  return 0;
}

extern "C" int dial_plan_observed_state(dial_plan* p, float* qpos, float* qvel, float* warm, int32_t* counters,
                                        int32_t* age, void* stream) {
  static const char* fn = "dial_plan_observed_state";
  if (!p) return fail(std::string(fn) + ": null plan");
  if (!p->mpc_bound) return fail(std::string(fn) + ": call dial_mpc_bind first");
  const size_t B = (size_t)p->n_inst, nq = p->hM.m.nq, nv = p->hM.m.nv;
  const bool ob = p->ran.obs;
  cudaStream_t st = (cudaStream_t)stream;
  const auto cp = [&](void* dst, const void* src, size_t bytes) {
    return dst ? cudaMemcpyAsync(dst, src, bytes, cudaMemcpyDeviceToDevice, st) : cudaSuccess;
  };
  CUDA_OK(cp(qpos, ob ? p->ob.oq : p->mpc.qpos, B * nq * sizeof(float)));
  CUDA_OK(cp(qvel, ob ? p->ob.ov : p->mpc.qvel, B * nv * sizeof(float)));
  CUDA_OK(cp(warm, ob ? p->ob.ow : p->mpc.qacc_warmstart, B * nv * sizeof(float)));
  CUDA_OK(cp(counters, ob ? p->ob.oc : p->mpc.counters, B * 2 * sizeof(int32_t)));
  if (age) {
    if (ob) CUDA_OK(cp(age, p->ob.age, B * sizeof(int32_t)));
    else CUDA_OK(cudaMemsetAsync(age, 0, B * sizeof(int32_t), st));
  }
  return 0;
}

extern "C" int dial_plan_pending_actions(dial_plan* p, float* out, void* stream) {
  static const char* fn = "dial_plan_pending_actions";
  if (!p || !out) return fail(std::string(fn) + ": null argument");
  const size_t n = (size_t)p->n_inst * DIAL_MAXDELAY * p->hM.m.nu * sizeof(float);
  cudaStream_t st = (cudaStream_t)stream;
  if (p->queue.pending) CUDA_OK(cudaMemcpyAsync(out, p->queue.pending, n, cudaMemcpyDeviceToDevice, st));
  else CUDA_OK(cudaMemsetAsync(out, 0, n, st));
  return 0;
}

extern "C" int dial_plan_planning_state(dial_plan* p, float* qpos, float* qvel, float* warm, int32_t* counters, void* stream) {
  static const char* fn = "dial_plan_planning_state";
  if (!p) return fail(std::string(fn) + ": null plan");
  if (!p->mpc_bound) return fail(std::string(fn) + ": call dial_mpc_bind first");
  const size_t B = (size_t)p->n_inst, nq = p->hM.m.nq, nv = p->hM.m.nv;
  const bool pred = p->ran.planning();
  cudaStream_t st = (cudaStream_t)stream;
  const auto cp = [&](void* dst, const void* src, size_t bytes) {
    return dst ? cudaMemcpyAsync(dst, src, bytes, cudaMemcpyDeviceToDevice, st) : cudaSuccess;
  };
  const dial_plan::PlanningState& P = p->planning;
  CUDA_OK(cp(qpos, pred ? P.qpos : p->mpc.qpos, B * nq * sizeof(float)));
  CUDA_OK(cp(qvel, pred ? P.qvel : p->mpc.qvel, B * nv * sizeof(float)));
  CUDA_OK(cp(warm, pred ? P.warm : p->mpc.qacc_warmstart, B * nv * sizeof(float)));
  CUDA_OK(cp(counters, pred ? P.cnt : p->mpc.counters, B * 2 * sizeof(int32_t)));
  return 0;
}

extern "C" int dial_plan_get_task(const dial_plan* p, dial_task* out) {
  if (!p || !out) return fail("dial_plan_get_task: null argument");
  const dial_task& t = plan_task(p->hP.c);
  if (!task_valid(t)) return fail("dial_plan_get_task: the plan's n_stage / n_user are out of range (1..DIAL_MAXSTAGE / 0..DIAL_MAXUSER)");
  *out = t;
  return 0;
}

extern "C" int dial_env_step(dial_plan* p, const dial_state* s, const float* action, float* qpos_out,
                             float* qvel_out, float* warm_out, float* reward, float* ctrl_out, void* stream) {
  return dial_env_step_kin(p, s, action, qpos_out, qvel_out, warm_out, reward, ctrl_out, nullptr, stream);
}

extern "C" int dial_env_step_kin(dial_plan* p, const dial_state* s, const float* action, float* qpos_out,
                                 float* qvel_out, float* warm_out, float* reward, float* ctrl_out, float* kin_out,
                                 void* stream) {
  if (!p || !s || !action || !qpos_out || !qvel_out || !warm_out || !reward) return fail("dial_env_step: null argument");
  RolloutArgs A; memset(&A, 0, sizeof(A));
  fill_state(A, s);
  A.nrows = 1; A.H = 1; A.mode = 0; A.us = action; A.rewss = reward;
  A.qpos_out = qpos_out; A.qvel_out = qvel_out; A.warm_out = warm_out; A.ctrl_out = ctrl_out; A.kin_out = kin_out;
  CUDA_OK(launch_rollout(p, A, 1, (cudaStream_t)stream));
  return 0;
}

extern "C" int dial_pipeline_init(dial_plan* p, const float* qpos, const float* qvel, float* qpos_out,
                                  float* warm_out, void* stream) {
  if (!p || !qpos || !qvel || !qpos_out || !warm_out) return fail("dial_pipeline_init: null argument");
  RolloutArgs A; memset(&A, 0, sizeof(A));
  A.qpos0 = qpos; A.qvel0 = qvel; A.warm0 = p->zeros;
  A.nrows = 1; A.H = 1; A.mode = 2; A.qpos_out = qpos_out; A.warm_out = warm_out;
  CUDA_OK(launch_rollout(p, A, 1, (cudaStream_t)stream));
  return 0;
}

extern "C" int dial_reverse_rollout(dial_plan* p, const dial_state* s, const float* eps, const uint32_t key[2],
                                    const float* Ybar, const float* noise_scale, float* rews_local, void* stream) {
  if (!p || !s || !Ybar || !noise_scale || !rews_local) return fail("dial_reverse_rollout: null argument");
  if (p->n_inst > 1) return fail("dial_reverse_rollout: batched plans run through dial_mpc_step");
  if (!eps && !key) return fail("dial_reverse_rollout: need eps or key");
  RolloutArgs A; memset(&A, 0, sizeof(A));
  fill_state(A, s);
  const dial_plan_desc& c = p->hP.c;
  A.nrows = c.Nsample + 1; A.H = c.Hsample + 1; A.mode = 1;
  A.eps = eps; A.Ybar = Ybar; A.noise = noise_scale;
  if (key) { A.key0 = key[0]; A.key1 = key[1]; }
  p->cur ^= 1;
  A.rews = rews_local; A.q = p->traj_q[p->cur]; A.qd = p->traj_qd[p->cur]; A.xpos = p->traj_x[p->cur];
  A.dbg = p->dbg;
  fill_xch(p, A);
  CUDA_OK(launch_rollout_any(p, A, (cudaStream_t)stream));
  return 0;
}

extern "C" int dial_reverse_update(dial_plan* p, const float* eps, const uint32_t key[2], const float* Ybar,
                                   const float* noise_scale, const float* rews_all, float* Ybar_out,
                                   float* weights, void* stream) {
  return dial_reverse_update_x(p, eps, key, Ybar, noise_scale, rews_all, Ybar_out, weights, nullptr, stream);
}

extern "C" int dial_reverse_update_x(dial_plan* p, const float* eps, const uint32_t key[2], const float* Ybar,
                                     const float* noise_scale, const float* rews_all, float* Ybar_out,
                                     float* weights, float* rews_gathered, void* stream) {
  if (!p || !Ybar || !noise_scale || !Ybar_out) return fail("dial_reverse_update: null argument");
  if (p->n_inst > 1) return fail("dial_reverse_update: batched plans run through dial_mpc_step");
  if (!rews_all && !p->xch.on) return fail("dial_reverse_update: rews_all may be NULL only with a connected exchange");
  if (!eps && !key) return fail("dial_reverse_update: need eps or key");
  const dial_plan_desc& c = p->hP.c;
  cudaStream_t st = (cudaStream_t)stream;
  float* w = weights ? weights : p->weights;
  XchWait X = xch_wait_args(p, rews_gathered);
  if (rews_all) X.mbox = nullptr;
  weights_kernel<<<1, 1024, 0, st>>>(rews_all, c.Ntotal + 1, c.temp_sample, w, X);
  p->launches++;
  CUDA_OK(cudaGetLastError());
  ybar_kernel<<<p->ybar_grid, YBAR_THREADS, 0, st>>>(w, eps, key ? key[0] : 0u, key ? key[1] : 0u, Ybar, noise_scale,
                                                     c.Ntotal, c.Hnode + 1, p->hM.m.nu, p->partial, p->counter, Ybar_out, nullptr);
  p->launches++;
  CUDA_OK(cudaGetLastError());
  if (weights && weights != p->weights)
    CUDA_OK(cudaMemcpyAsync(p->weights, weights, ((size_t)c.Ntotal + 1) * sizeof(float), cudaMemcpyDeviceToDevice, st));
  return 0;
}

static int launch_update(dial_plan* p, const float* rews, float* weights, const XchWait& X, uint32_t* rng,
                         const float* Ybar, const float* noise, float* Ybar_out, cudaStream_t st,
                         const InstSchedule* sched = nullptr, const int32_t* iter_lim = nullptr, int iter = 0,
                         const float* weights_prev = nullptr) {
  const dial_plan_desc& c = p->hP.c;
  update_kernel<<<dim3(p->upd_grid, p->n_inst), YBAR_THREADS, 0, st>>>(rews, c.Ntotal + 1, c.temp_sample, weights, X, rng, Ybar,
                                                                     noise, c.Ntotal, c.Hnode + 1, p->hM.m.nu, p->partial,
                                                                     p->counter, Ybar_out, sched, iter_lim, iter,
                                                                     weights_prev ? weights_prev : weights);
  p->launches++;
  CUDA_OK(cudaGetLastError());
  return 0;
}

extern "C" int dial_reverse_update_fused(dial_plan* p, const float* rews, uint32_t* rng, const float* Ybar,
                                         const float* noise_scale, float* Ybar_out, float* weights, void* stream) {
  if (!p || !rews || !rng || !Ybar || !noise_scale || !Ybar_out || !weights) return fail("dial_reverse_update_fused: null argument");
  const dial_plan_desc& c = p->hP.c;
  if (c.Ntotal != c.Nsample) return fail("dial_reverse_update_fused: sharded plans (Ntotal != Nsample) are not supported");
  if (c.Ntotal + 1 > (1 << 17)) return fail("dial_reverse_update_fused: needs Ntotal + 1 <= 131072 (the fused update)");
  XchWait X; memset(&X, 0, sizeof(X));
  return launch_update(p, rews, weights, X, rng, Ybar, noise_scale, Ybar_out, (cudaStream_t)stream);
}

static int enqueue_trajbar(dial_plan* p, const float* weights, int rank, float* qbar, float* qdbar, float* xbar,
                           cudaStream_t st, const int32_t* iter_lim = nullptr, int iter = 0) {
  const dial_plan_desc& c = p->hP.c;
  const dial_model_desc& m = p->hM.m;
  const float* w = weights ? weights : p->weights;
  const int H = c.Hsample + 1, rows = c.Nsample + 1;
  TrajArgs T;
  T.traj[0] = p->traj_q[p->cur]; T.traj[1] = p->traj_qd[p->cur]; T.traj[2] = p->traj_x[p->cur];
  T.out[0] = qbar; T.out[1] = qdbar; T.out[2] = xbar;
  const bool xsum = p->xch.on && qbar && qdbar && xbar;
  if (xsum) {
    T.out[0] = p->xch.bars_partial; T.out[1] = T.out[0] + (size_t)H * m.nq; T.out[2] = T.out[1] + (size_t)H * m.nv;
  }
  T.ncol[0] = m.nq; T.ncol[1] = m.nv; T.ncol[2] = 3 * (m.nbody - 1);
  T.coloff[0] = 0; T.coloff[1] = m.nq; T.coloff[2] = m.nq + m.nv;
  T.coltot = m.nq + m.nv + 3 * (m.nbody - 1);
  T.nrows = rows; T.inst_rows = (p->n_ens > 1 ? p->n_ens : 1) * rows; T.H = H; T.weights = w; T.w_offset = c.shard_offset; T.mean_row = c.Nsample;
  T.mean_weight_index = c.Ntotal; T.include_mean = rank == 0 ? 1 : 0; T.partial = p->tb_partial;
  const int maxlen = H * (T.ncol[2] > T.ncol[0] ? T.ncol[2] : T.ncol[0]);
  const dim3 g1((maxlen + 255) / 256, TB_CHUNKS, 3 * p->n_inst), g2(H, p->n_inst);
  const bool batch = p->n_inst > 1 || iter_lim;
  if (batch) trajbar_partial_kernel<true><<<g1, 256, 0, st>>>(T, iter_lim, iter);
  else trajbar_partial_kernel<false><<<g1, 256, 0, st>>>(T, nullptr, 0);
  p->launches++;
  CUDA_OK(cudaGetLastError());
  if (batch) trajbar_final_kernel<true><<<g2, 128, 0, st>>>(T, iter_lim, iter);
  else trajbar_final_kernel<false><<<g2, 128, 0, st>>>(T, nullptr, 0);
  p->launches++;
  CUDA_OK(cudaGetLastError());
  if (xsum) {
    BarsXch Bx; memset(&Bx, 0, sizeof(Bx));
    for (int r = 0; r < p->xch.world; ++r) { Bx.mbox[r] = p->xch.bars(r); Bx.flags[r] = p->xch.bflags(r); }
    Bx.seq = p->xch.bseq(); Bx.err = p->xch.err(); Bx.world = p->xch.world; Bx.rank = p->xch.rank; Bx.nbar = p->xch.nbar;
    Bx.partial = p->xch.bars_partial; Bx.out[0] = qbar; Bx.out[1] = qdbar; Bx.out[2] = xbar;
    Bx.n0 = H * m.nq; Bx.n1 = H * m.nv;
    bars_allreduce_kernel<<<1, 1024, 0, st>>>(Bx);
    p->launches++;
    CUDA_OK(cudaGetLastError());
  }
  return 0;
}

extern "C" int dial_reverse_trajbar(dial_plan* p, const float* weights, int rank, float* qbar, float* qdbar,
                                    float* xbar, void* stream) {
  if (!p) return fail("dial_reverse_trajbar: null plan");
  if (p->n_inst > 1) return fail("dial_reverse_trajbar: batched plans run through dial_mpc_step");
  return enqueue_trajbar(p, weights, rank, qbar, qdbar, xbar, (cudaStream_t)stream);
}

extern "C" int dial_exchange_create(dial_plan* p, int rank, int world, unsigned char handle_out[DIAL_IPC_HANDLE_BYTES]) {
  if (!p || !handle_out) return fail("dial_exchange_create: null argument");
  if (world < 2 || world > DIAL_MAXRANK || rank < 0 || rank >= world) return fail("dial_exchange_create: need 2 <= world <= DIAL_MAXRANK");
  static_assert(sizeof(cudaIpcMemHandle_t) <= DIAL_IPC_HANDLE_BYTES, "IPC handle does not fit");
  const dial_plan_desc& c = p->hP.c;
  const dial_model_desc& m = p->hM.m;
  if (c.Ntotal != c.Nsample * world || c.shard_offset != rank * c.Nsample) return fail("dial_exchange_create: plan shard does not match rank/world");
  if (p->xch.base[p->xch.rank]) return fail("dial_exchange_create: already created");
  dial_plan::Exchange& x = p->xch;
  x.rank = rank; x.world = world;
  x.nbar = (c.Hsample + 1) * (m.nq + m.nv + 3 * (m.nbody - 1));
  auto up = [](size_t n) { return (n + 31) & ~(size_t)31; };
  size_t o = 0;
  x.o_mbox = o; o += up(2 * ((size_t)c.Ntotal + 1));
  x.o_bars = o; o += up(2 * (size_t)DIAL_MAXRANK * x.nbar);
  x.o_flags = o; o += up(2 * DIAL_MAXRANK);
  x.o_bflags = o; o += up(2 * DIAL_MAXRANK);
  x.o_local = o; o += 32;
  x.words = o;
  void* d = nullptr;
  CUDA_OK(cudaMalloc(&d, x.words * sizeof(uint32_t)));
  CUDA_OK(cudaMemset(d, 0, x.words * sizeof(uint32_t)));
  x.base[rank] = reinterpret_cast<uint32_t*>(d);
  CUDA_OK(cudaMalloc(&x.bars_partial, (size_t)x.nbar * sizeof(float)));
  cudaIpcMemHandle_t h;
  CUDA_OK(cudaIpcGetMemHandle(&h, d));
  memset(handle_out, 0, DIAL_IPC_HANDLE_BYTES);
  memcpy(handle_out, &h, sizeof(h));
  return 0;
}

extern "C" int dial_exchange_connect(dial_plan* p, const unsigned char* handles) {
  if (!p || !handles) return fail("dial_exchange_connect: null argument");
  dial_plan::Exchange& x = p->xch;
  if (!x.base[x.rank]) return fail("dial_exchange_connect: call dial_exchange_create first");
  for (int r = 0; r < x.world; ++r) {
    if (r == x.rank) continue;
    cudaIpcMemHandle_t h;
    memcpy(&h, handles + (size_t)r * DIAL_IPC_HANDLE_BYTES, sizeof(h));
    void* d = nullptr;
    CUDA_OK(cudaIpcOpenMemHandle(&d, h, cudaIpcMemLazyEnablePeerAccess));
    x.base[r] = reinterpret_cast<uint32_t*>(d);
  }
  x.on = true;
  return 0;
}

extern "C" int dial_exchange_status(dial_plan* p, uint32_t out[6]) {
  if (!p || !out) return fail("dial_exchange_status: null argument");
  if (!p->xch.on) { for (int i = 0; i < 6; ++i) out[i] = 0; return 0; }
  CUDA_OK(cudaMemcpy(out, p->xch.base[p->xch.rank] + p->xch.o_local, 6 * sizeof(uint32_t), cudaMemcpyDeviceToHost));
  return 0;
}

extern "C" int dial_reverse_trajectories(dial_plan* p, float* q, float* qd, float* xpos, void* stream) {
  if (!p) return fail("dial_reverse_trajectories: null plan");
  if (p->n_inst > 1) return fail("dial_reverse_trajectories: batched plans run through dial_mpc_step");
  const dial_plan_desc& c = p->hP.c;
  const dial_model_desc& m = p->hM.m;
  const size_t n = ((size_t)c.Nsample + 1) * (c.Hsample + 1) * sizeof(float);
  cudaStream_t st = (cudaStream_t)stream;
  if (q) CUDA_OK(cudaMemcpyAsync(q, p->traj_q[p->cur], n * m.nq, cudaMemcpyDeviceToDevice, st));
  if (qd) CUDA_OK(cudaMemcpyAsync(qd, p->traj_qd[p->cur], n * m.nv, cudaMemcpyDeviceToDevice, st));
  if (xpos) CUDA_OK(cudaMemcpyAsync(xpos, p->traj_x[p->cur], n * 3 * (m.nbody - 1), cudaMemcpyDeviceToDevice, st));
  return 0;
}

extern "C" int dial_mpc_bind(dial_plan* p, const dial_mpc_buffers* b, const float* M_shift) {
  if (!p || !b || !M_shift) return fail("dial_mpc_bind: null argument");
  if (!b->qpos || !b->qvel || !b->qacc_warmstart || !b->counters || !b->rng || !b->Y || !b->ctrl || !b->reward ||
      !b->rews || !b->noise)
    return fail("dial_mpc_bind: only qbar/qdbar/xbar may be null");
  const dial_plan_desc& c = p->hP.c;
  if (c.Ntotal != c.Nsample && !p->xch.on)
    return fail("dial_mpc_bind: a sharded plan needs a connected exchange (dial_exchange_create / dial_exchange_connect) for the device-resident loop");
  if (c.Ntotal != c.Nsample && !b->rews_all) return fail("dial_mpc_bind: sharded plans need rews_all [Ntotal+1]");
  if (p->n_inst > 1 && b->rews_all) return fail("dial_mpc_bind: rews_all must be NULL on a batched plan");
  const int n1 = c.Hnode + 1, nu = p->hM.m.nu;
  drop_graphs(p);
  cudaError_t e = cudaSuccess;
  if (!p->mpc_Msh) CUDA_OK(p->own(e, p->mpc_Msh, DIAL_MAXNODE * DIAL_MAXNODE * sizeof(float)));
  if (!p->mpc_Y1) CUDA_OK(p->own(e, p->mpc_Y1, (size_t)p->n_inst * DIAL_MAXNODE * DIAL_MAXU * sizeof(float)));
  if (!p->mpc_key) CUDA_OK(p->own(e, p->mpc_key, 2 * sizeof(uint32_t)));
  CUDA_OK(cudaMemcpy(p->mpc_Msh, M_shift, (size_t)n1 * n1 * sizeof(float), cudaMemcpyHostToDevice));
  (void)nu;
  p->mpc = *b;
  p->mpc_bound = true;
  return 0;
}

static int mpc_enqueue(dial_plan* p, const LaunchKey& k, int n_diffuse, int env_step, cudaStream_t st) {
  const dial_plan_desc& c = p->hP.c;
  const dial_mpc_buffers& B = p->mpc;
  const int n1 = c.Hnode + 1, nu = p->hM.m.nu, ni = p->n_inst;
  const int K = p->n_ens > 1 ? p->n_ens : 1;
  const bool batched = ni > 1;
  const dial_plan::DelayQueue& Q = p->queue;
  const dial_plan::PlanningState& P = p->planning;
  float* Y[2] = {B.Y, p->mpc_Y1};
  int cur = 0;
  if (k.delay && (env_step == 1 || k.predicts)) {
    delay_queue_kernel<<<ni, 128, 0, st>>>(p->delay.d, Q.head, Q.ring, Y[cur], n1, nu, env_step == 1,
                                           Q.applied, Q.pending, Q.len);
    p->launches++;
    CUDA_OK(cudaGetLastError());
  }
  const float* act = k.delay ? Q.applied : Y[cur];
  const int act_n1 = k.delay ? 1 : n1;
  const bool adapt = env_step == 1 && k.adapt;
  if (adapt) {
    ens_gather_kernel<<<ni, 128, 0, st>>>(act, K, act_n1, nu, p->pred_us);
    p->launches++;
    CUDA_OK(cudaGetLastError());
    RolloutArgs A; memset(&A, 0, sizeof(A));
    A.qpos0 = B.qpos; A.qvel0 = B.qvel; A.warm0 = B.qacc_warmstart; A.counters_in = B.counters;
    A.nrows = ni * K; A.H = 1; A.mode = 0; A.us = p->pred_us;
    A.rows_per_inst = K; A.rows_per_model = 1; A.models = p->members.d;
    if (B.tasks) { A.tasks = B.tasks; A.task_rows = K; }
    A.qd = p->pred_qd;
    CUDA_OK(launch_rollout(p, A, 1, st));
  }
  if (env_step == 1) {
    RolloutArgs A; memset(&A, 0, sizeof(A));
    A.qpos0 = B.qpos; A.qvel0 = B.qvel; A.warm0 = B.qacc_warmstart;
    A.counters_in = B.counters; A.counters_out = B.counters;
    A.nrows = ni; A.H = 1; A.mode = 0; A.us = act; A.rewss = B.reward;
    if (batched) { A.rows_per_inst = 1; A.us_row = act_n1 * nu; }
    if (B.tasks) { A.tasks = B.tasks; A.task_rows = batched ? 1 : 0; }
    A.models = p->models.d;
    A.qpos_out = B.qpos; A.qvel_out = B.qvel; A.warm_out = B.qacc_warmstart; A.ctrl_out = B.ctrl;
    CUDA_OK(launch_rollout(p, A, 1, st));
  }
  if (adapt) {
    ens_belief_kernel<<<ni, 32, 0, st>>>(p->pred_qd, B.qvel, p->adapt.d, K, p->hM.m.nv, p->belief_L.d, p->belief_w.d, p->dEll);
    p->launches++;
    CUDA_OK(cudaGetLastError());
  }
  if (env_step == 1 || env_step == 2) {
    mpc_shift_kernel<<<ni, DIAL_MAXNODE * DIAL_MAXU, 0, st>>>(p->mpc_Msh, Y[cur], Y[cur ^ 1], n1, nu);
    p->launches++;
    CUDA_OK(cudaGetLastError());
    cur ^= 1;
  }
  const float *qpos0 = B.qpos, *qvel0 = B.qvel, *warm0 = B.qacc_warmstart;
  const int32_t* cnt0 = B.counters;
  if (k.obs) {
    observe_kernel<<<ni, 128, 0, st>>>(p->dM, p->obs.d, p->ob, p->delay.d, Q.pending, env_step == 1, B.qpos, B.qvel,
                                       B.qacc_warmstart, B.counters, act, act_n1 * nu, P.qpos, P.qvel, P.warm, P.cnt);
    p->launches++;
    CUDA_OK(cudaGetLastError());
  } else if (k.npred > 0) {
    const size_t nq = p->hM.m.nq, nv = p->hM.m.nv;
    CUDA_OK(cudaMemcpyAsync(P.qpos, B.qpos, ni * nq * sizeof(float), cudaMemcpyDeviceToDevice, st));
    CUDA_OK(cudaMemcpyAsync(P.qvel, B.qvel, ni * nv * sizeof(float), cudaMemcpyDeviceToDevice, st));
    CUDA_OK(cudaMemcpyAsync(P.warm, B.qacc_warmstart, ni * nv * sizeof(float), cudaMemcpyDeviceToDevice, st));
    CUDA_OK(cudaMemcpyAsync(P.cnt, B.counters, ni * 2 * sizeof(int32_t), cudaMemcpyDeviceToDevice, st));
  }
  for (int j = 0; j < k.npred; ++j) {
    RolloutArgs A; memset(&A, 0, sizeof(A));
    A.qpos0 = P.qpos; A.qvel0 = P.qvel; A.warm0 = P.warm;
    A.counters_in = P.cnt; A.counters_out = P.cnt;
    A.nrows = ni; A.H = 1; A.mode = 0; A.rows_per_inst = 1;
    A.us = (k.obs ? p->ob.seq : Q.pending) + (size_t)j * nu; A.us_row = DIAL_MAXDELAY * nu;
    if (B.tasks) { A.tasks = B.tasks; A.task_rows = batched ? 1 : 0; }
    A.models = p->n_ens > 0 ? P.models : p->models.d;
    A.iter_lim = k.obs ? p->ob.len : Q.len; A.iter = j;
    A.qpos_out = P.qpos; A.qvel_out = P.qvel; A.warm_out = P.warm;
    CUDA_OK(launch_rollout(p, A, 1, st));
  }
  if (k.planning()) { qpos0 = P.qpos; qvel0 = P.qvel; warm0 = P.warm; cnt0 = P.cnt; }
  const bool bars = B.qbar && B.qdbar && B.xbar;
  float* wts[2] = {p->weights, p->weights2};
  const size_t nw = (size_t)ni * (c.Ntotal + 1);
  for (int i = 0; i < n_diffuse; ++i) {
    const float* noise = B.noise + (size_t)i * n1;
    const bool fused = c.Ntotal + 1 <= (1 << 17) && !getenv("DIAL_NO_FUSED_UPDATE");
    if (!fused) {
      mpc_split_kernel<<<1, 32, 0, st>>>(B.rng, p->mpc_key);
      p->launches++;
      CUDA_OK(cudaGetLastError());
    }
    if (bars && i >= 2) CUDA_OK(cudaStreamWaitEvent(st, p->ev_side[i & 1], 0));
    RolloutArgs A; memset(&A, 0, sizeof(A));
    A.qpos0 = qpos0; A.qvel0 = qvel0; A.warm0 = warm0; A.counters_in = cnt0;
    A.nrows = ni * K * (c.Nsample + 1); A.H = c.Hsample + 1; A.mode = 1;
    if (batched || p->n_ens > 0) A.rows_per_inst = K * (c.Nsample + 1);
    if (B.tasks) { A.tasks = B.tasks; A.task_rows = batched ? K * (c.Nsample + 1) : 0; }
    if (p->n_ens > 0) { A.rows_per_model = c.Nsample + 1; A.models = p->members.d; }
    else A.models = p->models.d;
    A.Ybar = Y[cur]; A.noise = noise;
    A.sched = p->sched.d; A.iter_lim = p->lims.d; A.iter = i;
    if (fused) A.rng_dev = B.rng; else A.key_dev = p->mpc_key;
    p->cur ^= 1;
    A.rews = K > 1 ? p->ens_rews : B.rews; A.q = p->traj_q[p->cur]; A.qd = p->traj_qd[p->cur]; A.xpos = p->traj_x[p->cur];
    A.dbg = p->dbg;
    fill_xch(p, A);
    CUDA_OK(launch_rollout_any(p, A, st));
    if (K > 1) {
      const dim3 grid((c.Nsample + 1 + 255) / 256, ni);
      ensemble_reduce_kernel<<<grid, 256, 0, st>>>(p->ens_rews, p->risk.d, p->adapt.d, p->belief_w.d, K, c.Nsample + 1, B.rews,
                                                   p->lims.d, i);
      p->launches++;
      CUDA_OK(cudaGetLastError());
    }
    float* w = wts[i & 1];
    XchWait X = xch_wait_args(p, B.rews_all);
    if (fused) {
      int rc = launch_update(p, B.rews, w, X, B.rng, Y[cur], noise, Y[cur ^ 1], st, p->sched.d, p->lims.d, i,
                             wts[i > 0 ? (i - 1) & 1 : 0]);
      if (rc) return rc;
    } else {
      weights_kernel<<<1, 1024, 0, st>>>(B.rews, c.Ntotal + 1, c.temp_sample, w, X);
      p->launches++;
      CUDA_OK(cudaGetLastError());
      ybar_kernel<<<p->ybar_grid, YBAR_THREADS, 0, st>>>(w, nullptr, 0u, 0u, Y[cur], noise, c.Ntotal, n1, nu,
                                                         p->partial, p->counter, Y[cur ^ 1], p->mpc_key);
      p->launches++;
      CUDA_OK(cudaGetLastError());
    }
    cur ^= 1;
    if (bars) {
      CUDA_OK(cudaEventRecord(p->ev_main[i & 1], st));
      CUDA_OK(cudaStreamWaitEvent(p->side, p->ev_main[i & 1], 0));
      int rc = enqueue_trajbar(p, w, p->xch.on ? p->xch.rank : 0, B.qbar, B.qdbar, B.xbar, p->side, p->lims.d, i);
      if (rc) return rc;
      CUDA_OK(cudaEventRecord(p->ev_side[i & 1], p->side));
    }
  }
  if (cur != 0) CUDA_OK(cudaMemcpyAsync(Y[0], Y[1], (size_t)ni * n1 * nu * sizeof(float), cudaMemcpyDeviceToDevice, st));
  if (bars && n_diffuse > 0) {
    if (n_diffuse >= 2) CUDA_OK(cudaStreamWaitEvent(st, p->ev_side[(n_diffuse - 2) & 1], 0));
    CUDA_OK(cudaStreamWaitEvent(st, p->ev_side[(n_diffuse - 1) & 1], 0));
  }
  if (n_diffuse > 0 && wts[(n_diffuse - 1) & 1] != p->weights)
    CUDA_OK(cudaMemcpyAsync(p->weights, p->weights2, nw * sizeof(float), cudaMemcpyDeviceToDevice, st));
  return 0;
}

extern "C" int dial_mpc_step(dial_plan* p, int n_diffuse, int env_step, void* stream) {
  if (!p) return fail("dial_mpc_step: null plan");
  if (!p->mpc_bound) return fail("dial_mpc_step: call dial_mpc_bind first");
  if (n_diffuse < 0 || n_diffuse > 64) return fail("dial_mpc_step: n_diffuse out of range");
  if (env_step < 0 || env_step > 2) return fail("dial_mpc_step: env_step must be 0 (plan only), 1 (env step + shift) or 2 (shift only)");
  if (p->n_inst > 1 && getenv("DIAL_NO_FUSED_UPDATE")) return fail("dial_mpc_step: batched plans need the fused update (unset DIAL_NO_FUSED_UPDATE)");
  if ((p->sched.d || p->lims.d) && getenv("DIAL_NO_FUSED_UPDATE"))
    return fail("dial_mpc_step: per-instance schedules and iteration limits need the fused update (unset DIAL_NO_FUSED_UPDATE)");
  for (int b = 0; p->sched.d && b < p->n_inst; ++b) {
    const InstSchedule& S = p->sched.h[b];
    const int runs = p->lims.d && p->lims.h[b] < n_diffuse ? p->lims.h[b] : n_diffuse;
    if (S.on && runs > S.n_rows)
      return fail("dial_mpc_step: instance " + std::to_string(b) + " runs " + std::to_string(runs) +
                  " diffusion iterations, its schedule has " + std::to_string(S.n_rows) + " rows");
  }
  cudaStream_t st = (cudaStream_t)stream;
  if (p->key != p->ran) drop_graphs(p);
  p->ran = p->key;
  dial_plan::MpcGraph* g = nullptr;
  for (auto& e : p->mpc_graphs) if (e.n_diffuse == n_diffuse && e.env_step == env_step) g = &e;
  if (!g) {
    p->mpc_graphs.push_back({n_diffuse, env_step, 1, nullptr, 0});
    return mpc_enqueue(p, p->ran, n_diffuse, env_step, st);
  }
  if (!g->exec) {
    if (getenv("DIAL_NO_GRAPH")) return mpc_enqueue(p, p->ran, n_diffuse, env_step, st);
    cudaStream_t cs;
    CUDA_OK(cudaStreamCreateWithFlags(&cs, cudaStreamNonBlocking));
    const int64_t l0 = p->launches;
    cudaError_t e = cudaStreamBeginCapture(cs, cudaStreamCaptureModeThreadLocal);
    if (e != cudaSuccess) { cudaStreamDestroy(cs); CUDA_OK(e); }
    int rc = mpc_enqueue(p, p->ran, n_diffuse, env_step, cs);
    cudaGraph_t graph = nullptr;
    e = cudaStreamEndCapture(cs, &graph);
    cudaStreamDestroy(cs);
    g->launches = p->launches - l0;
    p->launches = l0;
    if (rc) { if (graph) cudaGraphDestroy(graph); return rc; }
    CUDA_OK(e);
    e = cudaGraphInstantiate(&g->exec, graph, 0);
    cudaGraphDestroy(graph);
    CUDA_OK(e);
  }
  CUDA_OK(cudaGraphLaunch(g->exec, st));
  p->launches += g->launches;
  return 0;
}

extern "C" void dial_key_split(const uint32_t key[2], uint32_t out0[2], uint32_t out1[2]) {
  uint32_t a0 = 0, b0 = 2, a1 = 1, b1 = 3;
  threefry2x32(key[0], key[1], a0, b0);
  threefry2x32(key[0], key[1], a1, b1);
  out0[0] = a0; out0[1] = a1; out1[0] = b0; out1[1] = b1;
}

extern "C" int dial_solver_variant(const dial_model_desc* model) {
  if (!model) return fail("null descriptor");
  DevModel* D = new (std::nothrow) DevModel();
  if (!D) return fail("out of memory");
  std::string err;
  int v = -1;
  if (!derive_model(*model, *D, err)) g_err = err;
  else if ((v = star_variant(*D)) < 0) g_err = "this build instantiates the dense (elliptic) solver path for nv = " DIAL_STR(DIAL_DENSE_NV) " only (custom builds: dial_mpc_b200.custom compiles it for the model's nv)";
  delete D;
  return v;
}

extern "C" const char* dial_plan_rollout_kernel(const dial_plan* p) {
  static const char* const generic[] = {"v0", "v1", "v2", "v3", "v4"};
  if (!p) return "";
#ifndef DIAL_ONLY_VARIANT
  if (p->shape > 0) return kShapes[p->shape - 1].name;
#endif
  return p->variant >= 0 && p->variant <= 4 ? generic[p->variant] : "";
}

extern "C" const char* dial_custom_reward_id(void) {
#if defined(DIAL_CUSTOM_REWARD_FILE) && defined(DIAL_CUSTOM_REWARD_ID)
  return DIAL_STR(DIAL_CUSTOM_REWARD_ID);
#elif defined(DIAL_CUSTOM_REWARD_FILE)
  return "custom";
#else
  return "";
#endif
}

__global__ void __launch_bounds__(1024) fp32_peak_kernel(float* out, int iters, float a, float b) {
  float x[8];
#pragma unroll
  for (int i = 0; i < 8; ++i) x[i] = (float)(threadIdx.x + i) * 1e-3f;
  for (int it = 0; it < iters; ++it) {
#pragma unroll
    for (int r = 0; r < 16; ++r) {
#pragma unroll
      for (int i = 0; i < 8; ++i) x[i] = fmaf(x[i], a, b);
    }
  }
  float s = 0.f;
#pragma unroll
  for (int i = 0; i < 8; ++i) s += x[i];
  if (s == 123.456f) out[0] = s;
}

extern "C" int dial_fp32_peak(int iters, float* tflops_out) {
  if (!tflops_out || iters < 1) return fail("dial_fp32_peak: bad argument");
  int dev = 0, sms = 0;
  CUDA_OK(cudaGetDevice(&dev));
  CUDA_OK(cudaDeviceGetAttribute(&sms, cudaDevAttrMultiProcessorCount, dev));
  float* d = nullptr;
  CUDA_OK(cudaMalloc(&d, sizeof(float)));
  cudaEvent_t e0, e1;
  CUDA_OK(cudaEventCreate(&e0));
  CUDA_OK(cudaEventCreate(&e1));
  const int grid = sms * 2;
  fp32_peak_kernel<<<grid, 1024>>>(d, 64, 0.999f, 1e-3f);
  float best = 0.f;
  for (int rep = 0; rep < 3; ++rep) {
    cudaEventRecord(e0);
    fp32_peak_kernel<<<grid, 1024>>>(d, iters, 0.999f, 1e-3f);
    cudaEventRecord(e1);
    cudaError_t e = cudaEventSynchronize(e1);
    if (e != cudaSuccess) { cudaFree(d); return fail(std::string("fp32 peak kernel: ") + cudaGetErrorString(e)); }
    float ms = 0.f;
    cudaEventElapsedTime(&ms, e0, e1);
    const double flop = 2.0 * 8 * 16 * (double)iters * 1024.0 * grid;
    const float tf = (float)(flop / (ms * 1e-3) / 1e12);
    best = tf > best ? tf : best;
  }
  cudaEventDestroy(e0); cudaEventDestroy(e1); cudaFree(d);
  *tflops_out = best;
  return 0;
}

extern "C" int64_t dial_launch_count(const dial_plan* p) { return p ? p->launches : 0; }
extern "C" int dial_rollout_wpc(const dial_plan* p, int nrows) { return (p && nrows > 0) ? default_wpc(p, nrows) : 0; }

extern "C" int dial_debug_counters(dial_plan* p, float out[8]) {
  if (!p || !p->dbg) return fail("debug counters are off (set DIAL_DEBUG_COUNTERS=1 before dial_plan_create)");
  CUDA_OK(cudaMemcpy(out, p->dbg, 8 * sizeof(float), cudaMemcpyDeviceToHost));
  CUDA_OK(cudaMemset(p->dbg, 0, 8 * sizeof(float)));
  return 0;
}
```

### dial_mpc_b200/csrc/dial_rollout_variant.cu

```cuda
#include <cuda_runtime.h>
#include "dial_host.h"

#ifndef DIAL_VARIANT
#error "compile with -DDIAL_VARIANT=<0..4>"
#endif
#if DIAL_VARIANT == 1
#define DIAL_V_NL 3
#define DIAL_V_NR 6
#elif DIAL_VARIANT == 2
#define DIAL_V_NL 5
#define DIAL_V_NR 7
#elif DIAL_VARIANT == 3
#define DIAL_V_NL -1
#define DIAL_V_NR DIAL_DENSE_NV
#elif DIAL_VARIANT == 4
#define DIAL_V_NL 5
#define DIAL_V_NR 6
#else
#define DIAL_V_NL 0
#define DIAL_V_NR 0
#endif

__device__ __forceinline__ uint32_t smem_u32(const void* p) { return (uint32_t)__cvta_generic_to_shared(p); }
__device__ __forceinline__ void mbar_init(uint64_t* bar, int count) {
  asm volatile("mbarrier.init.shared::cta.b64 [%0], %1;" ::"r"(smem_u32(bar)), "r"(count));
  asm volatile("fence.mbarrier_init.release.cluster;" ::: "memory");
}
__device__ __forceinline__ void mbar_expect_tx(uint64_t* bar, uint32_t bytes) {
  asm volatile("mbarrier.arrive.expect_tx.shared::cta.b64 _, [%0], %1;" ::"r"(smem_u32(bar)), "r"(bytes) : "memory");
}
__device__ __forceinline__ void tma_bulk_g2s(void* dst, const void* src, uint32_t bytes, uint64_t* bar) {
  asm volatile("cp.async.bulk.shared::cluster.global.mbarrier::complete_tx::bytes [%0], [%1], %2, [%3];"
               ::"r"(smem_u32(dst)), "l"(src), "r"(bytes), "r"(smem_u32(bar)) : "memory");
}
__device__ __forceinline__ void mbar_wait(uint64_t* bar, uint32_t parity) {
  asm volatile(
      "{\n .reg .pred p;\n WAIT_%=:\n"
      " mbarrier.try_wait.parity.shared::cta.b64 p, [%0], %1;\n"
      " @p bra DONE_%=;\n bra WAIT_%=;\n DONE_%=:\n}\n" ::"r"(smem_u32(bar)), "r"(parity) : "memory");
}

static_assert(sizeof(DevModel) % 16 == 0, "DevModel must be a multiple of 16 bytes for cp.async.bulk");
static_assert(sizeof(DevPlan) % 16 == 0, "DevPlan must be a multiple of 16 bytes for cp.async.bulk");

template <int NL, int NR, class SH = ShapeRT>
__global__ void __launch_bounds__(DIAL_MAXTHREADS, 1) rollout_kernel(const DevModel* __restrict__ gM,
                                                         const DevPlan* __restrict__ gP,
                                                         const RolloutArgs A) {
  extern __shared__ __align__(128) unsigned char smem[];
  __shared__ __align__(8) uint64_t bar;
  DevModel* sM = reinterpret_cast<DevModel*>(smem);
  DevPlan* sP = reinterpret_cast<DevPlan*>(smem + sizeof(DevModel));
  float* slabs = reinterpret_cast<float*>(smem + sizeof(DevModel) + sizeof(DevPlan));
  const int warp = threadIdx.x >> 5, lane = threadIdx.x & 31, wpc = blockDim.x >> 5;
  if (A.iter_lim && !schedule_runs(A.iter_lim, cta_instance(A, blockIdx.x, wpc), A.iter)) return;
  if (threadIdx.x == 0) {
    if (A.models) gM = A.models + (model_rows(A) > 0 ? blockIdx.x / ((model_rows(A) + wpc - 1) / wpc) : 0);
    mbar_init(&bar, 1);
    mbar_expect_tx(&bar, (uint32_t)(sizeof(DevModel) + sizeof(DevPlan)));
    tma_bulk_g2s(sM, gM, (uint32_t)sizeof(DevModel), &bar);
    tma_bulk_g2s(sP, gP, (uint32_t)sizeof(DevPlan), &bar);
  }
  __syncthreads();
  mbar_wait(&bar, 0);
  float* slab = slabs + (size_t)warp * sM->warp_floats;
  if constexpr (NL < 0) {
    if (A.row_counter) {
      for (;;) {
        int row = 0;
        if (lane == 0) row = (int)atomicAdd(A.row_counter, 1u);
        row = __shfl_sync(0xffffffffu, row, 0);
        if (row >= A.nrows) return;
        rollout_warp<NL, NR>(sM, sP, slab, A, row, lane);
        __syncwarp();
      }
    }
  }
  int row = blockIdx.x * wpc + warp;
  bool active = true;
  if (A.models && model_rows(A) > 0) {
    const int rps = model_rows(A), cpi = (rps + wpc - 1) / wpc, slot = blockIdx.x / cpi;
    row = (blockIdx.x - slot * cpi) * wpc + warp;
    if (row >= rps) {
      active = A.lockstep != 0;
      row = rps - 1;
    }
    row += slot * rps;
  }
  if (row >= A.nrows) {
    active = A.lockstep != 0;
    row = A.nrows - 1;
  }
  if (active) rollout_warp<NL, NR, SH>(sM, sP, slab, A, row, lane);
#ifndef DIAL_NO_XCH
  if (A.xch_world > 1) {
    __syncthreads();
    if (threadIdx.x == 0) {
      __threadfence_system();
      const unsigned int old = atomicAdd(A.xch_done, 1u);
      if (old == gridDim.x - 1) {
        __threadfence_system();
        const uint32_t seq = *A.xch_seq, buf = seq & 1u;
        for (int p = 0; p < A.xch_world; ++p)
          *reinterpret_cast<volatile uint32_t*>(A.xch_flags[p] + buf * DIAL_MAXRANK + A.xch_rank) = seq + 1u;
        *A.xch_done = 0u;
        __threadfence_system();
      }
    }
  }
#endif
}

#define DIAL_CAT2(a, b) a##b
#define DIAL_CAT(a, b) DIAL_CAT2(a, b)

#ifdef DIAL_SHAPE_NAME
#define DIAL_V_SHAPE ShapeFixed
#define DIAL_V_LAUNCHER DIAL_CAT(dial_launch_rollout_, DIAL_SHAPE_NAME)
bool DIAL_CAT(dial_shape_matches_, DIAL_SHAPE_NAME)(const DevModel& M, const dial_plan_desc& c) {
  return shape_matches<ShapeFixed>(M, c);
}
#else
#define DIAL_V_SHAPE ShapeRT
#define DIAL_V_LAUNCHER DIAL_CAT(dial_launch_rollout_v, DIAL_VARIANT)
#endif

cudaError_t DIAL_V_LAUNCHER(const DevModel* dM, const DevPlan* dP, const RolloutArgs& A,
                            int grid, int wpc, size_t smem, cudaStream_t st) {
  static size_t configured[64] = {0};
  int dev = 0;
  cudaError_t e = cudaGetDevice(&dev);
  if (e != cudaSuccess) return e;
  if (dev < 0 || dev >= 64 || smem > configured[dev]) {
    e = cudaFuncSetAttribute(rollout_kernel<DIAL_V_NL, DIAL_V_NR, DIAL_V_SHAPE>, cudaFuncAttributeMaxDynamicSharedMemorySize, (int)smem);
    if (e != cudaSuccess) { (void)cudaGetLastError(); return e; }
    if (dev >= 0 && dev < 64) configured[dev] = smem;
  }
  rollout_kernel<DIAL_V_NL, DIAL_V_NR, DIAL_V_SHAPE><<<grid, wpc * 32, smem, st>>>(dM, dP, A);
  return cudaGetLastError();
}
```

### dial_mpc_b200/custom.py

```python
from __future__ import annotations

import hashlib
import os
import shutil
import subprocess
from typing import Optional

from dial_mpc_b200 import _capi

_HERE = os.path.dirname(os.path.abspath(__file__))
_ROOT = os.path.dirname(_HERE)
CSRC = os.path.join(_HERE, "csrc")
CACHE_DIR = os.path.join(_HERE, "_custom")

NVCC_FLAGS = ["-gencode", "arch=compute_90a,code=sm_90a", "-lineinfo", "-O3", "-std=c++17",
              "-use_fast_math", "-shared", "-Xcompiler", "-fPIC", "-cudart", "static"]


def _sources(reward_path: str):
    return [os.path.join(CSRC, f) for f in ("dial_kernels.cu", "dial_rollout_variant.cu", "dial_device.cuh", "dial_host.h")] + \
        [os.path.join(_ROOT, "include", "dial_b200.h"), os.path.join(_ROOT, "include", "dial_custom_reward.h"),
         reward_path]


def _tag(variant: int, dense_nv: Optional[int], defines=()) -> str:
    return (f"v{variant}" + (f"n{dense_nv}" if variant == 3 and dense_nv not in (None, 22) else "")
            + ("x" if defines else ""))


def reward_id(reward_path: str, variant: int, dense_nv: Optional[int] = None, defines=()) -> str:
    h = hashlib.sha256()
    for s in _sources(reward_path):
        h.update(open(s, "rb").read())
    h.update((" ".join(NVCC_FLAGS) + f" variant={_tag(variant, dense_nv)[1:]}"
              + "".join(f" -D{d}" for d in sorted(defines))).encode())
    return h.hexdigest()[:16]


def library_path(reward_path: str, variant: int, dense_nv: Optional[int] = None, defines=()) -> str:
    stem = os.path.splitext(os.path.basename(reward_path))[0]
    return os.path.join(CACHE_DIR, f"libdial_b200_{stem}_{_tag(variant, dense_nv, defines)}_"
                                   f"{reward_id(reward_path, variant, dense_nv, defines)}.so")


def solver_variant(model) -> int:
    md = _capi.fill_model_desc(model)
    if dense_nv(model) is not None:
        return 3
    v = _capi.lib().dial_solver_variant(md)
    if v < 0:
        raise RuntimeError(f"model not supported: {_capi.lib().dial_last_error().decode()}")
    return v


def dense_nv(model) -> Optional[int]:
    md = _capi.fill_model_desc(model)
    if int(md.cone) != 1:
        return None
    if not 1 <= int(md.nv) <= 32:
        raise RuntimeError("the dense solver keeps one matrix row per lane: nv <= 32")
    return int(md.nv)


def build_library(reward_path: str, model=None, variant: Optional[int] = None, force: bool = False,
                  verbose: bool = False, defines=()) -> str:
    defines = tuple(defines)
    reward_path = os.path.abspath(reward_path)
    if not os.path.exists(reward_path):
        raise FileNotFoundError(reward_path)
    if variant is None:
        if model is None:
            raise ValueError("pass the compiled model (or the solver variant) the library is for")
        variant = solver_variant(model)
    nvd = dense_nv(model) if (model is not None and variant == 3) else None
    out = library_path(reward_path, variant, nvd, defines)
    if os.path.exists(out) and not force:
        return out
    nvcc = shutil.which("nvcc") or "/usr/local/cuda/bin/nvcc"
    if not os.path.exists(nvcc):
        raise RuntimeError("nvcc not found: custom rewards are compiled CUDA, there is no fallback")
    os.makedirs(CACHE_DIR, exist_ok=True)
    tmp = out + f".tmp{os.getpid()}"
    cmd = [nvcc] + NVCC_FLAGS + [f'-DDIAL_CUSTOM_REWARD_FILE="{reward_path}"',
                                 f"-DDIAL_CUSTOM_REWARD_ID={reward_id(reward_path, variant, nvd, defines)}",
                                 f"-DDIAL_ONLY_VARIANT={variant}"] + ([f"-DDIAL_DENSE_NV={nvd}"] if nvd else []) + [f"-D{d}" for d in defines] + [
                                 "-o", tmp, os.path.join(CSRC, "dial_kernels.cu")]
    if verbose:
        print(" ".join(cmd))
    r = subprocess.run(cmd, capture_output=True, text=True)
    if r.returncode != 0:
        if os.path.exists(tmp):
            os.remove(tmp)
        raise RuntimeError(f"nvcc failed for {reward_path}:\n{r.stdout}\n{r.stderr}")
    os.replace(tmp, out)
    import glob
    stem = os.path.splitext(os.path.basename(reward_path))[0]
    for old in glob.glob(os.path.join(CACHE_DIR, f"libdial_b200_{stem}_{_tag(variant, nvd, defines)}_*.so")):
        if old != out:
            try:
                os.remove(old)
            except OSError:
                pass
    return out
```

Before: 75.80 million.

## Fuse rollout, weight update and trajectory averaging into one cooperative persistent kernel

Adds a cooperative control_step kernel that loops over diffusion iterations inside one launch. Each pass runs the rollout warps, the softmax-weighted Ybar update with grid-wide partial sums, and at the end the weighted trajectory average, using grid.sync instead of separate kernel launches. The shared update, softmax and trajbar helpers move into a common header, and the update loop is batched four samples at a time for more memory-level parallelism. This is meant to remove per-iteration launch and host overhead, at the cost of grid-wide barriers and the occupancy limits of a cooperative launch.

```diff
diff --git a/__graft_entry__.py b/__graft_entry__.py
--- a/__graft_entry__.py
+++ b/__graft_entry__.py
@@ -45,12 +45,14 @@
 def build_library(force: bool = False, extra=(), lib: str = LIB, objdir: str = OBJDIR) -> None:
     extra = list(extra)
     tag = " " + " ".join(extra)
-    hdrs = [os.path.join(CSRC, f) for f in ("dial_device.cuh", "dial_host.h")] + [os.path.join(ROOT, "include", "dial_b200.h")]
+    hdrs = [os.path.join(CSRC, f) for f in ("dial_device.cuh", "dial_host.h", "dial_update.cuh", "dial_tma.cuh")] + \
+        [os.path.join(ROOT, "include", "dial_b200.h")]
     var_src = os.path.join(CSRC, "dial_rollout_variant.cu")
+    step_src = os.path.join(CSRC, "dial_control_step.cu")
     abi_src = os.path.join(CSRC, "dial_kernels.cu")
     shapes = _shape_defines()
     shape_tag = "".join(f" {name}:" + ",".join(d) for name, d in shapes)
-    lib_digest = _digest(hdrs + [var_src, abi_src], tag + shape_tag)
+    lib_digest = _digest(hdrs + [var_src, step_src, abi_src], tag + shape_tag)
     if not (force or _stale(lib, lib_digest)):
         return
     nvcc = os.environ.get("NVCC", "/usr/local/cuda/bin/nvcc")
@@ -65,6 +67,9 @@
         flags = ["-DDIAL_VARIANT=1", f"-DDIAL_SHAPE_NAME={name}"] + [f"-D{d}" for d in defs]
         jobs.append((obj, _digest(hdrs + [var_src], " " + " ".join(flags) + tag),
                      [nvcc] + NVCC_FLAGS + extra + flags + ["-c", "-o", obj, var_src]))
+        obj = os.path.join(objdir, f"control_step_{name}.o")
+        jobs.append((obj, _digest(hdrs + [step_src], " " + " ".join(flags) + tag),
+                     [nvcc] + NVCC_FLAGS + extra + flags + ["-c", "-o", obj, step_src]))
     obj = os.path.join(objdir, "dial_kernels.o")
     jobs.append((obj, _digest(hdrs + [abi_src], tag), [nvcc] + NVCC_FLAGS + extra + ["-c", "-o", obj, abi_src]))
     running = [(o, d, subprocess.Popen(cmd)) for o, d, cmd in jobs if force or _stale(o, d)]
diff --git a/dial_mpc_b200/csrc/dial_control_step.cu b/dial_mpc_b200/csrc/dial_control_step.cu
--- /dev/null
+++ b/dial_mpc_b200/csrc/dial_control_step.cu
@@ -0,0 +1,138 @@
+#include <cuda_runtime.h>
+#include <cooperative_groups.h>
+#include "dial_host.h"
+#include "dial_tma.cuh"
+#include "dial_update.cuh"
+
+#if !defined(DIAL_SHAPE_NAME) || DIAL_VARIANT != 1
+#error "compile with -DDIAL_VARIANT=1 -DDIAL_SHAPE_NAME=<s> and the shape's -DDIAL_SHAPE_* values"
+#endif
+
+namespace cg = cooperative_groups;
+
+template <int NL, int NR, class SH>
+__global__ void __launch_bounds__(DIAL_MAXTHREADS, 1) control_step_kernel(const DevModel* __restrict__ gM,
+                                                                         const DevPlan* __restrict__ gP,
+                                                                         const RolloutArgs A, const StepArgs S, int wpc) {
+  extern __shared__ __align__(128) unsigned char smem[];
+  __shared__ __align__(8) uint64_t bar;
+  __shared__ volatile int s_iter;
+  __shared__ volatile int s_last;
+  DevModel* sM = reinterpret_cast<DevModel*>(smem);
+  DevPlan* sP = reinterpret_cast<DevPlan*>(smem + sizeof(DevModel));
+  float* slabs = reinterpret_cast<float*>(smem + sizeof(DevModel) + sizeof(DevPlan));
+  cg::grid_group grid = cg::this_grid();
+  const int tid = threadIdx.x, ne = S.Hn1 * S.nu;
+  if (tid == 0) {
+    mbar_init(&bar, 1);
+    mbar_expect_tx(&bar, (uint32_t)(sizeof(DevModel) + sizeof(DevPlan)));
+    tma_bulk_g2s(sM, gM, (uint32_t)sizeof(DevModel), &bar);
+    tma_bulk_g2s(sP, gP, (uint32_t)sizeof(DevPlan), &bar);
+    s_iter = 0;
+  }
+  if (blockIdx.x == 0) {
+    float y = 0.f;
+    if (S.Msh && tid < ne) y = shift_knot(S.Msh, S.Y, tid, S.Hn1, S.nu);
+    __syncthreads();
+    if (S.Msh && tid < ne) S.Y[tid] = y;
+    if (tid < S.Hn1) S.noise_cur[tid] = S.noise[tid];
+  }
+  __syncthreads();
+  mbar_wait(&bar, 0);
+  grid.sync();
+  float* red = slabs;
+  float* acc = slabs + 4 * 32;
+  float* zsh = acc + YBAR_THREADS;
+  const int nthreads = gridDim.x * blockDim.x, gtid = blockIdx.x * blockDim.x + tid;
+  for (;;) {
+    {
+      const int warp = tid >> 5, lane = tid & 31;
+      int row = blockIdx.x * wpc + warp;
+      bool active = warp < wpc;
+      if (row >= A.nrows) {
+        active = active && A.lockstep != 0;
+        row = A.nrows - 1;
+      }
+      if (active) rollout_warp<NL, NR, SH>(sM, sP, slabs + (size_t)warp * sM->warp_floats, A, row, lane);
+    }
+    grid.sync();
+    const int it = s_iter;
+    const bool last = it + 1 >= S.n_diffuse;
+    const float* noise = S.noise + (size_t)it * S.Hn1;
+    if (tid == 0) s_last = 0;
+    if (tid < YBAR_THREADS) {
+      const SubThreads g{tid, YBAR_THREADS};
+      const uint32_t r0 = __ldcg(S.rng), r1 = __ldcg(S.rng + 1);
+      for (int v = blockIdx.x; v < S.upd_grid; v += gridDim.x) {
+        update_partial(g, v, S.upd_grid, S.rews, S.Ntotal + 1, S.temp, S.weights, r0, r1, S.Y, noise, S.Ntotal, S.Hn1,
+                       S.nu, S.partial, red, acc);
+        __threadfence();
+        g.sync();
+        if (tid == 0 && atomicAdd(S.counter, 1u) == (unsigned)S.upd_grid - 1) s_last = 1;
+      }
+    }
+    __syncthreads();
+    if (s_last) {
+      __threadfence();
+      if (tid == 0) *zsh = ordered_column_sum(S.partial + ne, ne + 1, S.upd_grid, true);
+      const float tot = ordered_column_sum(S.partial + tid, ne + 1, S.upd_grid, tid < ne);
+      __syncthreads();
+      const float iz = 1.f / *zsh;
+      if (tid < ne) S.Y[tid] = tot * iz;
+      if (tid == 0) {
+        *S.counter = 0u;
+        uint32_t n0, n1;
+        split_rng(__ldcg(S.rng), __ldcg(S.rng + 1), n0, n1);
+        S.rng[0] = n0; S.rng[1] = n1;
+      }
+      if (!last && tid < S.Hn1) S.noise_cur[tid] = noise[S.Hn1 + tid];
+      if (last)
+        for (int i = tid; i <= S.Ntotal; i += blockDim.x) S.weights[i] = __ldcg(S.weights + i) * iz;
+    }
+    grid.sync();
+    if (!last) {
+      if (tid == 0) s_iter = it + 1;
+      continue;
+    }
+    const TrajArgs& T = S.T;
+    const int nb0 = (T.H * T.ncol[0] + 255) / 256, nb1 = (T.H * T.ncol[1] + 255) / 256, nb2 = (T.H * T.ncol[2] + 255) / 256;
+    const int nb = nb0 + nb1 + nb2;
+    for (int L = gtid; L < TB_CHUNKS * nb * 256; L += nthreads) {
+      const int q = L >> 8, chunk = q / nb, b = q - chunk * nb;
+      const int arr = b < nb0 ? 0 : (b < nb0 + nb1 ? 1 : 2);
+      const int bx = b - (arr == 0 ? 0 : (arr == 1 ? nb0 : nb0 + nb1));
+      trajbar_partial_at<false>(T, bx, chunk, arr, 0, L & 255);
+    }
+    grid.sync();
+    for (int L = gtid; L < T.H * T.coltot; L += nthreads) trajbar_final_at(T, 0, L / T.coltot, L % T.coltot);
+    break;
+  }
+}
+
+#define DIAL_CAT2(a, b) a##b
+#define DIAL_CAT(a, b) DIAL_CAT2(a, b)
+
+cudaError_t DIAL_CAT(dial_launch_control_step_, DIAL_SHAPE_NAME)(const DevModel* dM, const DevPlan* dP, const RolloutArgs& A,
+                                                                const StepArgs& S, int grid, int wpc, size_t smem,
+                                                                cudaStream_t st) {
+  static size_t configured[64] = {0};
+  int dev = 0;
+  cudaError_t e = cudaGetDevice(&dev);
+  if (e != cudaSuccess) return e;
+  if (dev < 0 || dev >= 64 || smem > configured[dev]) {
+    e = cudaFuncSetAttribute(control_step_kernel<3, 6, ShapeFixed>, cudaFuncAttributeMaxDynamicSharedMemorySize, (int)smem);
+    if (e != cudaSuccess) { (void)cudaGetLastError(); return e; }
+    if (dev >= 0 && dev < 64) configured[dev] = smem;
+  }
+  cudaLaunchConfig_t cfg = {};
+  cudaLaunchAttribute attr[1];
+  attr[0].id = cudaLaunchAttributeCooperative;
+  attr[0].val.cooperative = 1;
+  cfg.gridDim = dim3(grid);
+  cfg.blockDim = dim3(32 * (wpc < 8 ? 8 : wpc));
+  cfg.dynamicSmemBytes = smem;
+  cfg.stream = st;
+  cfg.attrs = attr;
+  cfg.numAttrs = 1;
+  return cudaLaunchKernelEx(&cfg, control_step_kernel<3, 6, ShapeFixed>, dM, dP, A, S, wpc);
+}
diff --git a/dial_mpc_b200/csrc/dial_kernels.cu b/dial_mpc_b200/csrc/dial_kernels.cu
--- a/dial_mpc_b200/csrc/dial_kernels.cu
+++ b/dial_mpc_b200/csrc/dial_kernels.cu
@@ -8,6 +8,7 @@
 #include <vector>
 #include <new>
 #include "dial_host.h"
+#include "dial_update.cuh"
 #define DIAL_STR2(x) #x
 #define DIAL_STR(x) DIAL_STR2(x)
 
@@ -40,92 +41,23 @@
 #endif
 #ifndef DIAL_ONLY_VARIANT
 typedef cudaError_t (*dial_launch_fn)(const DevModel*, const DevPlan*, const RolloutArgs&, int, int, size_t, cudaStream_t);
+typedef cudaError_t (*dial_step_fn)(const DevModel*, const DevPlan*, const RolloutArgs&, const StepArgs&, int, int, size_t,
+                                    cudaStream_t);
 #define DIAL_DECL_SHAPE(s) \
   cudaError_t dial_launch_rollout_##s(const DevModel*, const DevPlan*, const RolloutArgs&, int, int, size_t, cudaStream_t); \
   bool dial_shape_matches_##s(const DevModel&, const dial_plan_desc&);
+#define DIAL_DECL_STEP(s) \
+  cudaError_t dial_launch_control_step_##s(const DevModel*, const DevPlan*, const RolloutArgs&, const StepArgs&, int, int, \
+                                           size_t, cudaStream_t);
 DIAL_DECL_SHAPE(go2)
+DIAL_DECL_STEP(go2)
 static const struct {
   const char* name;
   dial_launch_fn launch;
   bool (*matches)(const DevModel&, const dial_plan_desc&);
-} kShapes[] = {{"go2", dial_launch_rollout_go2, dial_shape_matches_go2}};
-#endif
-
-template <typename T, int K>
-__device__ __forceinline__ void block_reduce(T (&v)[K], T* mx, T* red) {
-  const int lane = threadIdx.x & 31, wid = threadIdx.x >> 5, nw = blockDim.x >> 5;
-#pragma unroll
-  for (int o = 16; o > 0; o >>= 1) {
-#pragma unroll
-    for (int k = 0; k < K; ++k) v[k] += __shfl_xor_sync(0xffffffffu, v[k], o);
-    if (mx) *mx = fmax(*mx, __shfl_xor_sync(0xffffffffu, *mx, o));
-  }
-  __syncthreads();
-  if (lane == 0) {
-#pragma unroll
-    for (int k = 0; k < K; ++k) red[k * 32 + wid] = v[k];
-    if (mx) red[K * 32 + wid] = *mx;
-  }
-  __syncthreads();
-#pragma unroll
-  for (int k = 0; k < K; ++k) v[k] = lane < nw ? red[k * 32 + lane] : T(0);
-  if (mx) *mx = lane < nw ? red[K * 32 + lane] : T(-INFINITY);
-#pragma unroll
-  for (int o = 16; o > 0; o >>= 1) {
-#pragma unroll
-    for (int k = 0; k < K; ++k) v[k] += __shfl_xor_sync(0xffffffffu, v[k], o);
-    if (mx) *mx = fmax(*mx, __shfl_xor_sync(0xffffffffu, *mx, o));
-  }
-}
-
-struct SoftmaxParams {
-  float shift, inv, mx;
-  bool none;
-};
-__device__ __noinline__ SoftmaxParams reward_softmax_params_fp64(const float* __restrict__ rews, int n, float temp,
-                                                                 float rbar, float mean, float cnt, float* red_f) {
-  double* red = reinterpret_cast<double*>(red_f);
-  SoftmaxParams s;
-  s.none = false;
-  const double c = isfinite(mean) ? (double)rbar + (double)mean : 0.0;
-  double s1[1] = {0.0}, s2[1] = {0.0}, rmax = -INFINITY;
-  for (int i = threadIdx.x; i < n; i += blockDim.x) {
-    const float r = __ldcg(rews + i);
-    if (isfinite(r)) { const double d = (double)r - c; s1[0] += d; s2[0] += d * d; rmax = fmax(rmax, (double)r); }
-  }
-  block_reduce<double, 1>(s1, &rmax, red);
-  block_reduce<double, 1>(s2, nullptr, red);
-  const double m = s1[0] / (double)cnt, var64 = s2[0] / (double)cnt - m * m;
-  s.shift = (float)rmax;
-  s.mx = 0.f;
-  s.inv = var64 > 0.0 ? (float)fmin(1.0 / (sqrt(var64) * (double)temp), 3.4028234663852886e38) : 0.f;
-  return s;
-}
-__device__ __forceinline__ SoftmaxParams reward_softmax_params(const float* __restrict__ rews, int n, float temp,
-                                                               float* red) {
-  float rbar = __ldcg(rews + n - 1);
-  const bool rbar_finite = isfinite(rbar);
-  if (!rbar_finite) rbar = 0.f;
-  float st[3] = {0.f, 0.f, 0.f}, dmax = -INFINITY;
-  for (int i = threadIdx.x; i < n; i += blockDim.x) {
-    const float r = __ldcg(rews + i);
-    if (isfinite(r)) { const float d = r - rbar; st[0] += 1.f; st[1] += d; st[2] += d * d; dmax = fmaxf(dmax, d); }
-  }
-  block_reduce<float, 3>(st, &dmax, red);
-  SoftmaxParams s;
-  const float cnt = st[0];
-  s.none = cnt == 0.f;
-  const float mean = st[1] / fmaxf(cnt, 1.f);
-  const float var = st[2] / fmaxf(cnt, 1.f) - mean * mean;
-  const float sd = sqrtf(fmaxf(var, 0.f));
-  if (s.none || (rbar_finite && isfinite(st[2]) && fabsf(mean) <= 8.f * sd)) {
-    s.shift = rbar;
-    s.inv = (sd > 0.f) ? 1.f / sd / temp : 0.f;
-    s.mx = dmax * s.inv;
-    return s;
-  }
-  return reward_softmax_params_fp64(rews, n, temp, rbar, mean, cnt, red);
-}
+  dial_step_fn step;
+} kShapes[] = {{"go2", dial_launch_rollout_go2, dial_shape_matches_go2, dial_launch_control_step_go2}};
+#endif
 
 struct XchWait {
   const float* mbox;
@@ -170,7 +102,8 @@
     if (X.rews_copy)
       for (int i = tid; i < n; i += blockDim.x) X.rews_copy[i] = __ldcg(rews + i);
   }
-  const SoftmaxParams s = reward_softmax_params(rews, n, temp, red);
+  const CtaThreads g{tid, (int)blockDim.x};
+  const SoftmaxParams s = reward_softmax_params(rews, n, temp, red, g);
   if (s.none) {
     for (int i = tid; i < n; i += blockDim.x) weights[i] = (i == n - 1) ? 1.f : 0.f;
     if (X.mbox && tid == 0) *X.seq = *X.seq + 1u;
@@ -183,7 +116,7 @@
     weights[i] = e;
     z[0] += e;
   }
-  block_reduce<float, 1>(z, nullptr, red);
+  block_reduce<float, 1>(z, nullptr, red, g);
   const float iz = 1.f / z[0];
   for (int i = tid; i < n; i += blockDim.x) weights[i] *= iz;
   if (X.mbox && tid == 0) *X.seq = *X.seq + 1u;
@@ -226,22 +159,6 @@
   if (threadIdx.x == 0) *B.seq = seq + 1u;
 }
 
-__device__ __forceinline__ float ordered_column_sum(const float* __restrict__ col, int stride, unsigned count, bool on) {
-  float tot = 0.f;
-  if (!on) return tot;
-  unsigned b = 0;
-  for (; b + 16 <= count; b += 16) {
-    float v[16];
-#pragma unroll
-    for (int k = 0; k < 16; ++k) v[k] = __ldcg(col + (size_t)(b + k) * stride);
-#pragma unroll
-    for (int k = 0; k < 16; ++k) tot += v[k];
-  }
-  for (; b < count; ++b) tot += __ldcg(col + (size_t)b * stride);
-  return tot;
-}
-
-#define YBAR_THREADS 256
 __global__ void __launch_bounds__(YBAR_THREADS) ybar_kernel(const float* __restrict__ weights, const float* __restrict__ eps,
                                                              uint32_t key0, uint32_t key1, const float* __restrict__ Ybar,
                                                              const float* __restrict__ noise, int Ntotal, int Hn1, int nu,
@@ -317,42 +234,10 @@
     xch_wait_flags(X.flags + buf * DIAL_MAXRANK, seq + 1u, X.world, X.err, blockIdx.x == 0 ? X.err + 2 : nullptr);
     rews = X.mbox + (size_t)buf * n;
   }
-  uint32_t key0, key1;
   const uint32_t r0 = rng[0], r1 = rng[1];
-  split_key(r0, r1, key0, key1);
-  const SoftmaxParams sp = reward_softmax_params(rews, n, temp, red);
   const int ne = Hn1 * nu;
-  const int slots = YBAR_THREADS / ne;
-  const int slot = tid / ne, el = tid - slot * ne;
-  float a = 0.f, z = 0.f;
-  if (slot < slots) {
-    const int k = el / nu;
-    const float yb = Ybar[el], ns = noise[k];
-    const uint32_t ntot = (uint32_t)Ntotal * (uint32_t)ne;
-    for (int s_ = blockIdx.x * slots + slot; s_ <= Ntotal; s_ += gridDim.x * slots) {
-      const float r = __ldcg(rews + s_);
-      float e = isfinite(r) ? expf((r - sp.shift) * sp.inv - sp.mx) : 0.f;
-      if (sp.none) e = (s_ == Ntotal) ? 1.f : 0.f;
-      float y = yb;
-      if (s_ < Ntotal && k > 0) {
-        const uint32_t idx = (uint32_t)s_ * (uint32_t)ne + (uint32_t)el;
-        y = jax_normal_legacy(key0, key1, idx, ntot) * ns + yb;
-      }
-      y = fminf(fmaxf(y, -1.f), 1.f);
-      a += e * y;
-      if (el == 0) { z += e; weights[s_] = e; }
-    }
-  }
-  acc[tid] = a;
-  float zz[1] = {z};
-  block_reduce<float, 1>(zz, nullptr, red);
-  __syncthreads();
-  if (tid < ne) {
-    float s_ = 0.f;
-    for (int sl = 0; sl < slots; ++sl) s_ += acc[sl * ne + tid];
-    partial[blockIdx.x * (ne + 1) + tid] = s_;
-  }
-  if (tid == 0) partial[blockIdx.x * (ne + 1) + ne] = zz[0];
+  update_partial(CtaThreads{tid, YBAR_THREADS}, blockIdx.x, gridDim.x, rews, n, temp, weights, r0, r1, Ybar, noise, Ntotal,
+                 Hn1, nu, partial, red, acc);
   __threadfence();
   __syncthreads();
   if (tid == 0) is_last = (atomicAdd(counter, 1u) == gridDim.x - 1);
@@ -393,78 +278,21 @@
                                  float* __restrict__ Yout, int n1, int nu) {
   const int i = threadIdx.x;
   Yin += (size_t)blockIdx.x * n1 * nu; Yout += (size_t)blockIdx.x * n1 * nu;
-  if (i < n1 * nu) {
-    const int k = i / nu, a = i - k * nu;
-    float s = 0.f;
-    for (int j = 0; j < n1; ++j) s += Msh[k * n1 + j] * Yin[j * nu + a];
-    Yout[i] = s;
-  }
-}
-
-#define TB_CHUNKS 32
-struct TrajArgs {
-  const float* traj[3];
-  float* out[3];
-  int ncol[3], coloff[3];
-  int coltot, nrows, H;
-  int inst_rows;
-  const float* weights;
-  int w_offset, mean_row, mean_weight_index, include_mean;
-  float* partial;
-};
+  if (i < n1 * nu) Yout[i] = shift_knot(Msh, Yin, i, n1, nu);
+}
 
 template <bool BATCH>
 __global__ void __launch_bounds__(256, 8) trajbar_partial_kernel(const TrajArgs T, const int32_t* __restrict__ iter_lim, int iter) {
-  const int chunk = blockIdx.y, arr = BATCH ? blockIdx.z % 3 : blockIdx.z, inst = BATCH ? blockIdx.z / 3 : 0;
-  const int ncol = arr == 0 ? T.ncol[0] : (arr == 1 ? T.ncol[1] : T.ncol[2]), len = T.H * ncol;
-  const int coloff = arr == 0 ? T.coloff[0] : (arr == 1 ? T.coloff[1] : T.coloff[2]);
-  const int j = blockIdx.x * 256 + threadIdx.x;
-  if (blockIdx.x * 256 >= len || (BATCH && !schedule_runs(iter_lim, inst, iter))) return;
-  const float* __restrict__ traj = (arr == 0 ? T.traj[0] : (arr == 1 ? T.traj[1] : T.traj[2])) + (size_t)inst * T.inst_rows * len;
-  const float* wts = BATCH ? T.weights + (size_t)inst * (T.mean_weight_index + 1) : T.weights;
-  const int per = (T.nrows + TB_CHUNKS - 1) / TB_CHUNKS;
-  const int r0 = chunk * per, r1 = min(T.nrows, r0 + per);
-  const int jj = j < len ? j : len - 1;
-  float a = 0.f;
-  for (int r = r0; r < r1; r += 8) {
-    float wv[8], xv[8];
-#pragma unroll
-    for (int k = 0; k < 8; ++k) {
-      const int rr = r + k;
-      float wgt = 0.f;
-      if (rr < r1) {
-        if (rr == T.mean_row) wgt = T.include_mean ? wts[T.mean_weight_index] : 0.f;
-        else wgt = wts[T.w_offset + rr];
-      }
-      wv[k] = wgt;
-    }
-#pragma unroll
-    for (int k = 0; k < 8; ++k)
-      xv[k] = (wv[k] != 0.f) ? traj[(size_t)(r + k) * len + jj] : 0.f;
-#pragma unroll
-    for (int k = 0; k < 8; ++k) a += wv[k] * xv[k];
-  }
-  if (j < len) {
-    const int t = j / ncol, c = j - t * ncol;
-    T.partial[(((size_t)inst * TB_CHUNKS + chunk) * T.H + t) * T.coltot + coloff + c] = a;
-  }
+  const int arr = BATCH ? blockIdx.z % 3 : blockIdx.z, inst = BATCH ? blockIdx.z / 3 : 0;
+  if (BATCH && !schedule_runs(iter_lim, inst, iter)) return;
+  trajbar_partial_at<BATCH>(T, blockIdx.x, blockIdx.y, arr, inst, threadIdx.x);
 }
 
 template <bool BATCH>
 __global__ void __launch_bounds__(128, 8) trajbar_final_kernel(const TrajArgs T, const int32_t* __restrict__ iter_lim, int iter) {
   const int t = blockIdx.x, inst = BATCH ? blockIdx.y : 0;
   if (BATCH && !schedule_runs(iter_lim, inst, iter)) return;
-  const float* partial = T.partial + (size_t)inst * TB_CHUNKS * T.H * T.coltot;
-  for (int col = threadIdx.x; col < T.coltot; col += blockDim.x) {
-    float s = 0.f;
-#pragma unroll 8
-    for (int ch = 0; ch < TB_CHUNKS; ++ch) s += partial[((size_t)ch * T.H + t) * T.coltot + col];
-    float* out; int ncol, off;
-    if (col >= T.coloff[2]) { out = T.out[2]; ncol = T.ncol[2]; off = T.coloff[2]; }
-    else if (col >= T.coloff[1]) { out = T.out[1]; ncol = T.ncol[1]; off = T.coloff[1]; }
-    else { out = T.out[0]; ncol = T.ncol[0]; off = T.coloff[0]; }
-    if (out) out[((size_t)inst * T.H + t) * ncol + (col - off)] = s;
-  }
+  for (int col = threadIdx.x; col < T.coltot; col += blockDim.x) trajbar_final_at(T, inst, t, col);
 }
 
 __global__ void __launch_bounds__(256) ensemble_reduce_kernel(const float* __restrict__ r, const EnsRisk* __restrict__ risk,
@@ -650,6 +478,7 @@
   float* mpc_Msh = nullptr;
   float* mpc_Y1 = nullptr;
   uint32_t* mpc_key = nullptr;
+  float* noise_cur = nullptr;
   struct MpcGraph { int n_diffuse, env_step, seen; cudaGraphExec_t exec; int64_t launches; };
   std::vector<MpcGraph> mpc_graphs;
   LaunchKey key, ran;
@@ -791,8 +620,7 @@
   return (per_sm + waves - 1) / waves;
 }
 
-static cudaError_t launch_rollout_any(dial_plan* p, const RolloutArgs& A0, cudaStream_t st) {
-  RolloutArgs A = A0;
+static int rollout_policy(const dial_plan* p, RolloutArgs& A) {
   const char* f = getenv("DIAL_WPC");
   int wpc = f ? atoi(f) : 0;
   if (wpc == 0) {
@@ -802,7 +630,7 @@
       wpc = (model_rows(A) + cpi - 1) / cpi;
     }
   }
-  if (wpc < 1 || wpc > DIAL_MAXTHREADS / 32) return cudaErrorInvalidValue;
+  if (wpc < 1 || wpc > DIAL_MAXTHREADS / 32) return 0;
   A.lockstep = (wpc >= 2 && !getenv("DIAL_NO_LOCKSTEP")) ? 1 : 0;
   if (p->hM.dense && !A.lockstep && !A.models && A.nrows > wpc * p->num_sms && !getenv("DIAL_NO_DYNAMIC_ROWS")) A.row_counter = p->row_counter;
   const bool mid = getenv("DIAL_MIDSYNC") ? true : (getenv("DIAL_NO_MIDSYNC") ? false : (p->hM.dense || !p->hM.s_on));
@@ -810,6 +638,13 @@
   { const char* se = getenv("DIAL_SYNC_EVERY"); A.sync_every = se ? atoi(se) : 1; if (A.sync_every < 1) A.sync_every = 1; }
   const char* dl = getenv("DIAL_DENSE_LOCKSTEP");
   if (A.lockstep == 2 && p->hM.dense && !(dl && atoi(dl) == 2)) A.lockstep = 3;
+  return wpc;
+}
+
+static cudaError_t launch_rollout_any(dial_plan* p, const RolloutArgs& A0, cudaStream_t st) {
+  RolloutArgs A = A0;
+  const int wpc = rollout_policy(p, A);
+  if (wpc == 0) return cudaErrorInvalidValue;
   return launch_rollout(p, A, wpc, st);
 }
 
@@ -1479,24 +1314,31 @@
   return launch_update(p, rews, weights, X, rng, Ybar, noise_scale, Ybar_out, (cudaStream_t)stream);
 }
 
+static TrajArgs traj_args(const dial_plan* p, const float* weights, int rank, float* qbar, float* qdbar, float* xbar) {
+  const dial_plan_desc& c = p->hP.c;
+  const dial_model_desc& m = p->hM.m;
+  const int rows = c.Nsample + 1;
+  TrajArgs T;
+  T.traj[0] = p->traj_q[p->cur]; T.traj[1] = p->traj_qd[p->cur]; T.traj[2] = p->traj_x[p->cur];
+  T.out[0] = qbar; T.out[1] = qdbar; T.out[2] = xbar;
+  T.ncol[0] = m.nq; T.ncol[1] = m.nv; T.ncol[2] = 3 * (m.nbody - 1);
+  T.coloff[0] = 0; T.coloff[1] = m.nq; T.coloff[2] = m.nq + m.nv;
+  T.coltot = m.nq + m.nv + 3 * (m.nbody - 1);
+  T.nrows = rows; T.inst_rows = (p->n_ens > 1 ? p->n_ens : 1) * rows; T.H = c.Hsample + 1; T.weights = weights ? weights : p->weights;
+  T.w_offset = c.shard_offset; T.mean_row = c.Nsample;
+  T.mean_weight_index = c.Ntotal; T.include_mean = rank == 0 ? 1 : 0; T.partial = p->tb_partial;
+  return T;
+}
+
 static int enqueue_trajbar(dial_plan* p, const float* weights, int rank, float* qbar, float* qdbar, float* xbar,
                            cudaStream_t st, const int32_t* iter_lim = nullptr, int iter = 0) {
   const dial_plan_desc& c = p->hP.c;
   const dial_model_desc& m = p->hM.m;
-  const float* w = weights ? weights : p->weights;
-  const int H = c.Hsample + 1, rows = c.Nsample + 1;
-  TrajArgs T;
-  T.traj[0] = p->traj_q[p->cur]; T.traj[1] = p->traj_qd[p->cur]; T.traj[2] = p->traj_x[p->cur];
-  T.out[0] = qbar; T.out[1] = qdbar; T.out[2] = xbar;
+  const int H = c.Hsample + 1;
   const bool xsum = p->xch.on && qbar && qdbar && xbar;
-  if (xsum) {
-    T.out[0] = p->xch.bars_partial; T.out[1] = T.out[0] + (size_t)H * m.nq; T.out[2] = T.out[1] + (size_t)H * m.nv;
-  }
-  T.ncol[0] = m.nq; T.ncol[1] = m.nv; T.ncol[2] = 3 * (m.nbody - 1);
-  T.coloff[0] = 0; T.coloff[1] = m.nq; T.coloff[2] = m.nq + m.nv;
-  T.coltot = m.nq + m.nv + 3 * (m.nbody - 1);
-  T.nrows = rows; T.inst_rows = (p->n_ens > 1 ? p->n_ens : 1) * rows; T.H = H; T.weights = w; T.w_offset = c.shard_offset; T.mean_row = c.Nsample;
-  T.mean_weight_index = c.Ntotal; T.include_mean = rank == 0 ? 1 : 0; T.partial = p->tb_partial;
+  TrajArgs T = xsum ? traj_args(p, weights, rank, p->xch.bars_partial, p->xch.bars_partial + (size_t)H * m.nq,
+                                p->xch.bars_partial + (size_t)H * (m.nq + m.nv))
+                    : traj_args(p, weights, rank, qbar, qdbar, xbar);
   const int maxlen = H * (T.ncol[2] > T.ncol[0] ? T.ncol[2] : T.ncol[0]);
   const dim3 g1((maxlen + 255) / 256, TB_CHUNKS, 3 * p->n_inst), g2(H, p->n_inst);
   const bool batch = p->n_inst > 1 || iter_lim;
@@ -1611,10 +1453,50 @@
   if (!p->mpc_Msh) CUDA_OK(p->own(e, p->mpc_Msh, DIAL_MAXNODE * DIAL_MAXNODE * sizeof(float)));
   if (!p->mpc_Y1) CUDA_OK(p->own(e, p->mpc_Y1, (size_t)p->n_inst * DIAL_MAXNODE * DIAL_MAXU * sizeof(float)));
   if (!p->mpc_key) CUDA_OK(p->own(e, p->mpc_key, 2 * sizeof(uint32_t)));
+  if (!p->noise_cur) CUDA_OK(p->own(e, p->noise_cur, DIAL_MAXNODE * sizeof(float)));
   CUDA_OK(cudaMemcpy(p->mpc_Msh, M_shift, (size_t)n1 * n1 * sizeof(float), cudaMemcpyHostToDevice));
   (void)nu;
   p->mpc = *b;
   p->mpc_bound = true;
+  return 0;
+}
+
+static int enqueue_persistent_step(dial_plan* p, const LaunchKey& k, int n_diffuse, int env_step, bool bars, bool fused,
+                                   cudaStream_t st, bool* done) {
+  *done = false;
+#ifndef DIAL_ONLY_VARIANT
+  const dial_plan_desc& c = p->hP.c;
+  const dial_mpc_buffers& B = p->mpc;
+  if (p->shape == 0 || !kShapes[p->shape - 1].step || p->n_inst > 1 || p->n_ens > 0 || p->xch.on || c.Ntotal != c.Nsample ||
+      k.models || k.members || k.sched || k.lims || k.adapt || k.delay || k.obs || !bars || !fused || n_diffuse < 1 ||
+      getenv("DIAL_NO_PERSISTENT_STEP"))
+    return 0;
+  RolloutArgs A; memset(&A, 0, sizeof(A));
+  A.qpos0 = B.qpos; A.qvel0 = B.qvel; A.warm0 = B.qacc_warmstart; A.counters_in = B.counters;
+  A.nrows = c.Nsample + 1; A.H = c.Hsample + 1; A.mode = 1;
+  if (B.tasks) A.tasks = B.tasks;
+  A.Ybar = B.Y; A.noise = p->noise_cur; A.rng_dev = B.rng; A.rews = B.rews;
+  A.dbg = p->dbg;
+  const int wpc = rollout_policy(p, A);
+  const int grid = wpc > 0 ? (A.nrows + wpc - 1) / wpc : 0;
+  const size_t fixed = sizeof(DevModel) + sizeof(DevPlan), slabs = (size_t)wpc * p->hM.warp_floats * sizeof(float);
+  if (wpc == 0 || grid > p->num_sms || (A.lockstep && wpc < 8) || A.row_counter ||
+      slabs < (4 * 32 + YBAR_THREADS + 1) * sizeof(float))
+    return 0;
+  p->cur ^= n_diffuse & 1;
+  A.q = p->traj_q[p->cur]; A.qd = p->traj_qd[p->cur]; A.xpos = p->traj_x[p->cur];
+  StepArgs S;
+  S.Msh = env_step != 0 ? p->mpc_Msh : nullptr;
+  S.Y = B.Y; S.rng = B.rng; S.noise = B.noise; S.noise_cur = p->noise_cur; S.rews = B.rews; S.weights = p->weights;
+  S.partial = p->partial; S.counter = p->counter; S.temp = c.temp_sample; S.Ntotal = c.Ntotal; S.Hn1 = c.Hnode + 1; S.nu = p->hM.m.nu;
+  S.n_diffuse = n_diffuse; S.upd_grid = p->upd_grid;
+  S.T = traj_args(p, p->weights, 0, B.qbar, B.qdbar, B.xbar);
+  CUDA_OK(kShapes[p->shape - 1].step(p->dM, p->dP, A, S, grid, wpc, fixed + slabs, st));
+  p->launches++;
+  *done = true;
+#else
+  (void)p; (void)k; (void)n_diffuse; (void)env_step; (void)bars; (void)fused; (void)st;
+#endif
   return 0;
 }
 
@@ -1665,6 +1547,13 @@
     p->launches++;
     CUDA_OK(cudaGetLastError());
   }
+  const bool bars = B.qbar && B.qdbar && B.xbar;
+  const bool fused = c.Ntotal + 1 <= (1 << 17) && !getenv("DIAL_NO_FUSED_UPDATE");
+  {
+    bool done = false;
+    if (int rc = enqueue_persistent_step(p, k, n_diffuse, env_step, bars, fused, st, &done)) return rc;
+    if (done) return 0;
+  }
   if (env_step == 1 || env_step == 2) {
     mpc_shift_kernel<<<ni, DIAL_MAXNODE * DIAL_MAXU, 0, st>>>(p->mpc_Msh, Y[cur], Y[cur ^ 1], n1, nu);
     p->launches++;
@@ -1698,12 +1587,10 @@
     CUDA_OK(launch_rollout(p, A, 1, st));
   }
   if (k.planning()) { qpos0 = P.qpos; qvel0 = P.qvel; warm0 = P.warm; cnt0 = P.cnt; }
-  const bool bars = B.qbar && B.qdbar && B.xbar;
   float* wts[2] = {p->weights, p->weights2};
   const size_t nw = (size_t)ni * (c.Ntotal + 1);
   for (int i = 0; i < n_diffuse; ++i) {
     const float* noise = B.noise + (size_t)i * n1;
-    const bool fused = c.Ntotal + 1 <= (1 << 17) && !getenv("DIAL_NO_FUSED_UPDATE");
     if (!fused) {
       mpc_split_kernel<<<1, 32, 0, st>>>(B.rng, p->mpc_key);
       p->launches++;
diff --git a/dial_mpc_b200/csrc/dial_rollout_variant.cu b/dial_mpc_b200/csrc/dial_rollout_variant.cu
--- a/dial_mpc_b200/csrc/dial_rollout_variant.cu
+++ b/dial_mpc_b200/csrc/dial_rollout_variant.cu
@@ -1,5 +1,6 @@
 #include <cuda_runtime.h>
 #include "dial_host.h"
+#include "dial_tma.cuh"
 
 #ifndef DIAL_VARIANT
 #error "compile with -DDIAL_VARIANT=<0..4>"
@@ -20,28 +21,6 @@
 #define DIAL_V_NL 0
 #define DIAL_V_NR 0
 #endif
-
-__device__ __forceinline__ uint32_t smem_u32(const void* p) { return (uint32_t)__cvta_generic_to_shared(p); }
-__device__ __forceinline__ void mbar_init(uint64_t* bar, int count) {
-  asm volatile("mbarrier.init.shared::cta.b64 [%0], %1;" ::"r"(smem_u32(bar)), "r"(count));
-  asm volatile("fence.mbarrier_init.release.cluster;" ::: "memory");
-}
-__device__ __forceinline__ void mbar_expect_tx(uint64_t* bar, uint32_t bytes) {
-  asm volatile("mbarrier.arrive.expect_tx.shared::cta.b64 _, [%0], %1;" ::"r"(smem_u32(bar)), "r"(bytes) : "memory");
-}
-__device__ __forceinline__ void tma_bulk_g2s(void* dst, const void* src, uint32_t bytes, uint64_t* bar) {
-  asm volatile("cp.async.bulk.shared::cluster.global.mbarrier::complete_tx::bytes [%0], [%1], %2, [%3];"
-               ::"r"(smem_u32(dst)), "l"(src), "r"(bytes), "r"(smem_u32(bar)) : "memory");
-}
-__device__ __forceinline__ void mbar_wait(uint64_t* bar, uint32_t parity) {
-  asm volatile(
-      "{\n .reg .pred p;\n WAIT_%=:\n"
-      " mbarrier.try_wait.parity.shared::cta.b64 p, [%0], %1;\n"
-      " @p bra DONE_%=;\n bra WAIT_%=;\n DONE_%=:\n}\n" ::"r"(smem_u32(bar)), "r"(parity) : "memory");
-}
-
-static_assert(sizeof(DevModel) % 16 == 0, "DevModel must be a multiple of 16 bytes for cp.async.bulk");
-static_assert(sizeof(DevPlan) % 16 == 0, "DevPlan must be a multiple of 16 bytes for cp.async.bulk");
 
 template <int NL, int NR, class SH = ShapeRT>
 __global__ void __launch_bounds__(DIAL_MAXTHREADS, 1) rollout_kernel(const DevModel* __restrict__ gM,
diff --git a/dial_mpc_b200/csrc/dial_tma.cuh b/dial_mpc_b200/csrc/dial_tma.cuh
--- /dev/null
+++ b/dial_mpc_b200/csrc/dial_tma.cuh
@@ -0,0 +1,25 @@
+#pragma once
+#include <cuda_runtime.h>
+#include "dial_host.h"
+
+__device__ __forceinline__ uint32_t smem_u32(const void* p) { return (uint32_t)__cvta_generic_to_shared(p); }
+__device__ __forceinline__ void mbar_init(uint64_t* bar, int count) {
+  asm volatile("mbarrier.init.shared::cta.b64 [%0], %1;" ::"r"(smem_u32(bar)), "r"(count));
+  asm volatile("fence.mbarrier_init.release.cluster;" ::: "memory");
+}
+__device__ __forceinline__ void mbar_expect_tx(uint64_t* bar, uint32_t bytes) {
+  asm volatile("mbarrier.arrive.expect_tx.shared::cta.b64 _, [%0], %1;" ::"r"(smem_u32(bar)), "r"(bytes) : "memory");
+}
+__device__ __forceinline__ void tma_bulk_g2s(void* dst, const void* src, uint32_t bytes, uint64_t* bar) {
+  asm volatile("cp.async.bulk.shared::cluster.global.mbarrier::complete_tx::bytes [%0], [%1], %2, [%3];"
+               ::"r"(smem_u32(dst)), "l"(src), "r"(bytes), "r"(smem_u32(bar)) : "memory");
+}
+__device__ __forceinline__ void mbar_wait(uint64_t* bar, uint32_t parity) {
+  asm volatile(
+      "{\n .reg .pred p;\n WAIT_%=:\n"
+      " mbarrier.try_wait.parity.shared::cta.b64 p, [%0], %1;\n"
+      " @p bra DONE_%=;\n bra WAIT_%=;\n DONE_%=:\n}\n" ::"r"(smem_u32(bar)), "r"(parity) : "memory");
+}
+
+static_assert(sizeof(DevModel) % 16 == 0, "DevModel must be a multiple of 16 bytes for cp.async.bulk");
+static_assert(sizeof(DevPlan) % 16 == 0, "DevPlan must be a multiple of 16 bytes for cp.async.bulk");
diff --git a/dial_mpc_b200/csrc/dial_update.cuh b/dial_mpc_b200/csrc/dial_update.cuh
--- /dev/null
+++ b/dial_mpc_b200/csrc/dial_update.cuh
@@ -0,0 +1,247 @@
+#pragma once
+#include <float.h>
+#include "dial_host.h"
+
+struct CtaThreads {
+  int tid, n;
+  __device__ __forceinline__ void sync() const { __syncthreads(); }
+};
+struct SubThreads {
+  int tid, n;
+  __device__ __forceinline__ void sync() const { asm volatile("bar.sync 1, %0;" ::"r"(n) : "memory"); }
+};
+
+template <typename T, int K, class G>
+__device__ __forceinline__ void block_reduce(T (&v)[K], T* mx, T* red, const G& g) {
+  const int lane = g.tid & 31, wid = g.tid >> 5, nw = g.n >> 5;
+#pragma unroll
+  for (int o = 16; o > 0; o >>= 1) {
+#pragma unroll
+    for (int k = 0; k < K; ++k) v[k] += __shfl_xor_sync(0xffffffffu, v[k], o);
+    if (mx) *mx = fmax(*mx, __shfl_xor_sync(0xffffffffu, *mx, o));
+  }
+  g.sync();
+  if (lane == 0) {
+#pragma unroll
+    for (int k = 0; k < K; ++k) red[k * 32 + wid] = v[k];
+    if (mx) red[K * 32 + wid] = *mx;
+  }
+  g.sync();
+#pragma unroll
+  for (int k = 0; k < K; ++k) v[k] = lane < nw ? red[k * 32 + lane] : T(0);
+  if (mx) *mx = lane < nw ? red[K * 32 + lane] : T(-INFINITY);
+#pragma unroll
+  for (int o = 16; o > 0; o >>= 1) {
+#pragma unroll
+    for (int k = 0; k < K; ++k) v[k] += __shfl_xor_sync(0xffffffffu, v[k], o);
+    if (mx) *mx = fmax(*mx, __shfl_xor_sync(0xffffffffu, *mx, o));
+  }
+}
+
+struct SoftmaxParams {
+  float shift, inv, mx;
+  bool none;
+};
+template <class G>
+__device__ __noinline__ SoftmaxParams reward_softmax_params_fp64(const float* __restrict__ rews, int n, float temp,
+                                                                 float rbar, float mean, float cnt, float* red_f, const G g) {
+  double* red = reinterpret_cast<double*>(red_f);
+  SoftmaxParams s;
+  s.none = false;
+  const double c = isfinite(mean) ? (double)rbar + (double)mean : 0.0;
+  double s1[1] = {0.0}, s2[1] = {0.0}, rmax = -INFINITY;
+  for (int i = g.tid; i < n; i += g.n) {
+    const float r = __ldcg(rews + i);
+    if (isfinite(r)) { const double d = (double)r - c; s1[0] += d; s2[0] += d * d; rmax = fmax(rmax, (double)r); }
+  }
+  block_reduce<double, 1>(s1, &rmax, red, g);
+  block_reduce<double, 1>(s2, nullptr, red, g);
+  const double m = s1[0] / (double)cnt, var64 = s2[0] / (double)cnt - m * m;
+  s.shift = (float)rmax;
+  s.mx = 0.f;
+  s.inv = var64 > 0.0 ? (float)fmin(1.0 / (sqrt(var64) * (double)temp), 3.4028234663852886e38) : 0.f;
+  return s;
+}
+template <class G>
+__device__ __forceinline__ SoftmaxParams reward_softmax_params(const float* __restrict__ rews, int n, float temp,
+                                                               float* red, const G& g) {
+  float rbar = __ldcg(rews + n - 1);
+  const bool rbar_finite = isfinite(rbar);
+  if (!rbar_finite) rbar = 0.f;
+  float st[3] = {0.f, 0.f, 0.f}, dmax = -INFINITY;
+  for (int i = g.tid; i < n; i += g.n) {
+    const float r = __ldcg(rews + i);
+    if (isfinite(r)) { const float d = r - rbar; st[0] += 1.f; st[1] += d; st[2] += d * d; dmax = fmaxf(dmax, d); }
+  }
+  block_reduce<float, 3>(st, &dmax, red, g);
+  SoftmaxParams s;
+  const float cnt = st[0];
+  s.none = cnt == 0.f;
+  const float mean = st[1] / fmaxf(cnt, 1.f);
+  const float var = st[2] / fmaxf(cnt, 1.f) - mean * mean;
+  const float sd = sqrtf(fmaxf(var, 0.f));
+  if (s.none || (rbar_finite && isfinite(st[2]) && fabsf(mean) <= 8.f * sd)) {
+    s.shift = rbar;
+    s.inv = (sd > 0.f) ? 1.f / sd / temp : 0.f;
+    s.mx = dmax * s.inv;
+    return s;
+  }
+  return reward_softmax_params_fp64(rews, n, temp, rbar, mean, cnt, red, g);
+}
+
+__device__ __forceinline__ float ordered_column_sum(const float* __restrict__ col, int stride, unsigned count, bool on) {
+  float tot = 0.f;
+  if (!on) return tot;
+  unsigned b = 0;
+  for (; b + 16 <= count; b += 16) {
+    float v[16];
+#pragma unroll
+    for (int k = 0; k < 16; ++k) v[k] = __ldcg(col + (size_t)(b + k) * stride);
+#pragma unroll
+    for (int k = 0; k < 16; ++k) tot += v[k];
+  }
+  for (; b < count; ++b) tot += __ldcg(col + (size_t)b * stride);
+  return tot;
+}
+
+#define YBAR_THREADS 256
+
+template <class G>
+__device__ __forceinline__ void update_partial(const G& g, int cta, int ncta, const float* rews, int n, float temp,
+                                               float* weights, uint32_t r0, uint32_t r1, const float* Ybar,
+                                               const float* noise, int Ntotal, int Hn1, int nu, float* partial,
+                                               float* red, float* acc) {
+  const int tid = g.tid;
+  uint32_t key0, key1;
+  split_key(r0, r1, key0, key1);
+  const SoftmaxParams sp = reward_softmax_params(rews, n, temp, red, g);
+  const int ne = Hn1 * nu;
+  const int slots = YBAR_THREADS / ne;
+  const int slot = tid / ne, el = tid - slot * ne;
+  float a = 0.f, z = 0.f;
+  if (slot < slots) {
+    const int k = el / nu;
+    const float yb = __ldcg(Ybar + el), ns = noise[k];
+    const uint32_t ntot = (uint32_t)Ntotal * (uint32_t)ne;
+    constexpr int UPD_BATCH = 4;
+    const int stride = ncta * slots;
+    for (int s0 = cta * slots + slot; s0 <= Ntotal; s0 += UPD_BATCH * stride) {
+      float ev[UPD_BATCH], yv[UPD_BATCH];
+#pragma unroll
+      for (int j = 0; j < UPD_BATCH; ++j) {
+        const int s_ = s0 + j * stride;
+        ev[j] = 0.f; yv[j] = 0.f;
+        if (s_ > Ntotal) continue;
+        const float r = __ldcg(rews + s_);
+        float e = isfinite(r) ? expf((r - sp.shift) * sp.inv - sp.mx) : 0.f;
+        if (sp.none) e = (s_ == Ntotal) ? 1.f : 0.f;
+        float y = yb;
+        if (s_ < Ntotal && k > 0) {
+          const uint32_t idx = (uint32_t)s_ * (uint32_t)ne + (uint32_t)el;
+          y = jax_normal_legacy(key0, key1, idx, ntot) * ns + yb;
+        }
+        ev[j] = e; yv[j] = fminf(fmaxf(y, -1.f), 1.f);
+      }
+#pragma unroll
+      for (int j = 0; j < UPD_BATCH; ++j) {
+        const int s_ = s0 + j * stride;
+        if (s_ > Ntotal) break;
+        a += ev[j] * yv[j];
+        if (el == 0) { z += ev[j]; weights[s_] = ev[j]; }
+      }
+    }
+  }
+  acc[tid] = a;
+  float zz[1] = {z};
+  block_reduce<float, 1>(zz, nullptr, red, g);
+  g.sync();
+  if (tid < ne) {
+    float s_ = 0.f;
+    for (int sl = 0; sl < slots; ++sl) s_ += acc[sl * ne + tid];
+    partial[cta * (ne + 1) + tid] = s_;
+  }
+  if (tid == 0) partial[cta * (ne + 1) + ne] = zz[0];
+}
+
+__device__ __forceinline__ float shift_knot(const float* __restrict__ Msh, const float* Yin, int i, int n1, int nu) {
+  const int k = i / nu, a = i - k * nu;
+  float s = 0.f;
+  for (int j = 0; j < n1; ++j) s += Msh[k * n1 + j] * Yin[j * nu + a];
+  return s;
+}
+
+#define TB_CHUNKS 32
+struct TrajArgs {
+  const float* traj[3];
+  float* out[3];
+  int ncol[3], coloff[3];
+  int coltot, nrows, H;
+  int inst_rows;
+  const float* weights;
+  int w_offset, mean_row, mean_weight_index, include_mean;
+  float* partial;
+};
+
+template <bool BATCH>
+__device__ __forceinline__ void trajbar_partial_at(const TrajArgs& T, int bx, int chunk, int arr, int inst, int tid) {
+  const int ncol = arr == 0 ? T.ncol[0] : (arr == 1 ? T.ncol[1] : T.ncol[2]), len = T.H * ncol;
+  const int coloff = arr == 0 ? T.coloff[0] : (arr == 1 ? T.coloff[1] : T.coloff[2]);
+  const int j = bx * 256 + tid;
+  if (bx * 256 >= len) return;
+  const float* traj = (arr == 0 ? T.traj[0] : (arr == 1 ? T.traj[1] : T.traj[2])) + (size_t)inst * T.inst_rows * len;
+  const float* wts = BATCH ? T.weights + (size_t)inst * (T.mean_weight_index + 1) : T.weights;
+  const int per = (T.nrows + TB_CHUNKS - 1) / TB_CHUNKS;
+  const int r0 = chunk * per, r1 = min(T.nrows, r0 + per);
+  const int jj = j < len ? j : len - 1;
+  float a = 0.f;
+  for (int r = r0; r < r1; r += 8) {
+    float wv[8], xv[8];
+#pragma unroll
+    for (int k = 0; k < 8; ++k) {
+      const int rr = r + k;
+      float wgt = 0.f;
+      if (rr < r1) {
+        if (rr == T.mean_row) wgt = T.include_mean ? __ldcg(wts + T.mean_weight_index) : 0.f;
+        else wgt = __ldcg(wts + T.w_offset + rr);
+      }
+      wv[k] = wgt;
+    }
+#pragma unroll
+    for (int k = 0; k < 8; ++k)
+      xv[k] = (wv[k] != 0.f) ? __ldcg(traj + (size_t)(r + k) * len + jj) : 0.f;
+#pragma unroll
+    for (int k = 0; k < 8; ++k) a += wv[k] * xv[k];
+  }
+  if (j < len) {
+    const int t = j / ncol, c = j - t * ncol;
+    T.partial[(((size_t)inst * TB_CHUNKS + chunk) * T.H + t) * T.coltot + coloff + c] = a;
+  }
+}
+
+__device__ __forceinline__ void trajbar_final_at(const TrajArgs& T, int inst, int t, int col) {
+  const float* partial = T.partial + (size_t)inst * TB_CHUNKS * T.H * T.coltot;
+  float s = 0.f;
+#pragma unroll 8
+  for (int ch = 0; ch < TB_CHUNKS; ++ch) s += __ldcg(partial + ((size_t)ch * T.H + t) * T.coltot + col);
+  float* out; int ncol, off;
+  if (col >= T.coloff[2]) { out = T.out[2]; ncol = T.ncol[2]; off = T.coloff[2]; }
+  else if (col >= T.coloff[1]) { out = T.out[1]; ncol = T.ncol[1]; off = T.coloff[1]; }
+  else { out = T.out[0]; ncol = T.ncol[0]; off = T.coloff[0]; }
+  if (out) out[((size_t)inst * T.H + t) * ncol + (col - off)] = s;
+}
+
+struct StepArgs {
+  const float* Msh;
+  float* Y;
+  uint32_t* rng;
+  const float* noise;
+  float* noise_cur;
+  const float* rews;
+  float* weights;
+  float* partial;
+  unsigned int* counter;
+  float temp;
+  int Ntotal, Hn1, nu, n_diffuse;
+  int upd_grid;
+  TrajArgs T;
+};
diff --git a/dial_mpc_b200/custom.py b/dial_mpc_b200/custom.py
--- a/dial_mpc_b200/custom.py
+++ b/dial_mpc_b200/custom.py
@@ -18,7 +18,8 @@
 
 
 def _sources(reward_path: str):
-    return [os.path.join(CSRC, f) for f in ("dial_kernels.cu", "dial_rollout_variant.cu", "dial_device.cuh", "dial_host.h")] + \
+    return [os.path.join(CSRC, f) for f in ("dial_kernels.cu", "dial_rollout_variant.cu", "dial_device.cuh", "dial_host.h",
+                                            "dial_update.cuh", "dial_tma.cuh")] + \
         [os.path.join(_ROOT, "include", "dial_b200.h"), os.path.join(_ROOT, "include", "dial_custom_reward.h"),
          reward_path]
 
```

New measurement: 77.12 million, median of 6. +1.7%, better.
